# tonyckc/WT-PSE-code

Hardware: AMD Instinct MI355X
Metric: training images/sec (256x256 fundus) — full WT-PSE iteration (higher is better)
Workload: dtype f32 (layers with > 16 output channels and the fused 1x1 heads: x2h (2 fp16 terms per fp32 operand — power-of-two operand scaling —, 3 fp16 MFMA products per multiply, fp32 accumulation); the 16-channel layers the same on 16x16x32, the 1-/3-channel input layers and small 1x1 convs fp32-input MFMA)

## Files before the change

### include/wtpse_hip.h

```cpp
#ifndef WTPSE_HIP_H
#define WTPSE_HIP_H
#ifdef __cplusplus
extern "C" {
#endif


int wtpse_pack_conv_weights(const float* params, const int* desc, int n_desc, float* packed, void* stream);

int wtpse_conv_fwd(const float* in0, int C0, const float* in1, int C1, const float* wpacked, const float* bias,
                   const float* pro0, const float* pro1, int pro_relu, float* out0, float* out1, int Csplit, float* stats,
                   int B, int H, int W, int Cout, int ksize, int relu_out, const float* mask_ref, unsigned* out_amax, void* stream);
int wtpse_conv_stats_blocks(int B, int H, int W);
int wtpse_conv_fwd_gram(const float* in0, int C0, const float* wpacked, const float* bias, const float* pro0, int pro_relu,
                        float* out0, float* gram_partial, int B, int H, int W, int Cout, int relu_out, unsigned* out_amax,
                        void* stream);

int wtpse_conv_x3_stats_blocks(int B, int H, int W, int Cout, int ksize);
int wtpse_x3r_enable(int on);
int wtpse_x3_xcd(int on);
int wtpse_x3_small_wide(int on);
int wtpse_x3_terms(int terms);
int wtpse_amax(const float* x, long long n, unsigned* amax_table, void* stream);
int wtpse_pack_conv_weights_x3(const float* params, const int* desc, int n_desc, unsigned short* packed, void* stream);
int wtpse_conv_fwd_x3(const float* in0, int C0, const float* in1, int C1, const unsigned short* wpacked, const float* bias,
                      const float* pro0, const float* pro1, int pro_relu, float* out0, float* out1, int Csplit, float* stats,
                      int B, int H, int W, int Cout, int ksize, int relu_out, const float* mask_ref, const unsigned* in_amax,
                      const unsigned* in_amax1, unsigned* out_amax, void* stream);

int wtpse_conv16_x3(const float* in0, int C0, const unsigned short* wx16, const float* bias, const float* pro0, int pro_relu,
                    float* out0, float* stats, float* gram_partial, const float* mask_ref, const float* bn_ss,
                    const float* bn_mean, int bn_relu, int B, int H, int W, int Cout, int relu_out, int in_is_grad,
                    const unsigned* in_amax, unsigned* out_amax, void* stream);
int wtpse_pack_conv16_x3(const float* params, const int* desc, int n_desc, unsigned short* packed, void* stream);

int wtpse_dgrad_bnb(const float* dy, int C, const float* wpacked, float* out0, float* out1, int Csplit, const float* bn_y,
                    const float* bn_ss, const float* bn_mean, int bn_relu, int bn_c0, int bn_c1, float* stats, int B, int H, int W,
                    int Cout, int ksize, void* stream);
int wtpse_dgrad_x3_bnb(const float* dy, int C, const unsigned short* wpacked, float* out0, float* out1, int Csplit,
                       const float* bn_y, const float* bn_ss, const float* bn_mean, int bn_relu, int bn_c0, int bn_c1, float* stats,
                       int B, int H, int W, int Cout, int ksize, const unsigned* in_amax, void* stream);

int wtpse_conv_fwd_bnf(const float* in0, int C0, const float* in1, int C1, const void* wpacked, int layout, const float* bias,
                       const float* pro0, const float* pro1, int pro_relu, float* out0, float* stats, const float* gamma,
                       const float* beta, float* running_mean, float* running_var, long long* num_batches, float momentum, float eps,
                       float* scale_shift, float* save_mean, float* save_invstd, double* partial2, unsigned* tickets, int B, int H,
                       int W, int Cout, int ksize, const unsigned* in_amax0, const unsigned* in_amax1, unsigned* act_amax, void* stream);

int wtpse_bnb_tail_partial2(int nblk, int Cout);
int wtpse_bnb_tail_tickets(int nblk, int Cout);
int wtpse_dgrad_bnb_coef(const float* dy, int C, const void* wpacked, int layout, float* out0, float* out1, int Csplit,
                         const float* bn_y, const float* bn_ss, const float* bn_mean, int bn_relu, int bn_c0, int bn_c1,
                         float* stats, const float* gamma, const float* invstd, float* coef, float* dgamma, float* dbeta,
                         int accumulate, double* partial2, unsigned* tickets, int B, int H, int W, int Cout, int ksize,
                         const unsigned* in_amax, void* stream);
int wtpse_dgrad_bnb_coef_frozen(const float* dy, int C, const void* wpacked, int layout, float* out0, float* out1, int Csplit,
                                const float* bn_y, const float* bn_ss, const float* bn_mean, int bn_relu, int bn_c0, int bn_c1,
                                float* stats, const float* gamma, const float* invstd, float* coef, float* dgamma, float* dbeta,
                                float* dbias, int accumulate, double* partial2, unsigned* tickets, int B, int H, int W, int Cout,
                                int ksize, const unsigned* in_amax, void* stream);

int wtpse_conv_wgrad(const float* dy, const float* x0, int C0, const float* x1, int C1, const float* pro0,
                     const float* pro1, int pro_relu, float* slab, float* dbias_slab, int ksplit, float* dw, float* dbias, int accumulate, int B, int H,
                     int W, int Cout, int ksize, void* stream);
int wtpse_wgrad_ksplit(int B, int H, int W, int Cin, int Cout);
int wtpse_wgrad_x3_supported(int Cin, int Cout, int ksize, int C0);
int wtpse_wgrad_x3_ksplit(int B, int H, int W, int Cin, int Cout);
int wtpse_conv_wgrad_x3(const float* dy, const float* x0, int C0, const float* x1, int C1, const float* pro0,
                        const float* pro1, int pro_relu, float* slab, int ksplit, float* dw, int accumulate, int B, int H, int W,
                        int Cout, int ksize, void* stream);

int wtpse_wgrad_r_supported(int Cin, int Cout, int ksize, int C0, int W);
int wtpse_wgrad_r_slabs(int B, int H, int W, int Cin, int Cout);
int wtpse_conv_wgrad_r(const float* dy, const float* x0, int C0, const float* x1, int C1, const float* pro0,
                       const float* pro1, int pro_relu, float* slab, float* dbias_slab, int nslab, float* dw, float* dbias,
                       int accumulate, int B, int H, int W, int Cout, const unsigned* dy_amax, const unsigned* x_amax0,
                       const unsigned* x_amax1, void* stream);

int wtpse_conv_wgrad_r_bn(const float* g, const float* bn_y, const float* bn_coef, const float* x0, int C0, const float* x1,
                          int C1, const float* pro0, const float* pro1, int pro_relu, float* slab, int nslab, float* dw,
                          int accumulate, int B, int H, int W, int Cout, void* stream);

int wtpse_bn_finalize(const float* stats_partial, int nblk, int C, long long count, const float* gamma, const float* beta,
                      float* running_mean, float* running_var, long long* num_batches, float momentum, float eps,
                      float* scale_shift, float* save_mean, float* save_invstd, unsigned* act_amax, void* stream);
int wtpse_bn_finalize_blend(const float* stats_partial, int nblk, int C, long long count, const float* gamma, const float* beta,
                            const float* running_mean, const float* running_var, double w, float eps, double* acc, double acc_count,
                            float* scale_shift, double* moments, double* div, unsigned* act_amax, void* stream);
int wtpse_act_bound(const float* scale_shift, int C, const unsigned* raw_amax, unsigned* act_amax, void* stream);
int wtpse_bn_eval_coeffs(const float* gamma, const float* beta, const float* running_mean, const float* running_var,
                         float eps, int C, float* scale_shift, void* stream);
int wtpse_affine_act(const float* y, const float* scale_shift, int relu, float* z, int B, int C, int HW, void* stream);
int wtpse_bn_bwd(const float* dz, const float* y, const float* scale_shift, int relu, const float* gamma,
                 const float* save_mean, const float* save_invstd, float* partial, float* coef, float* dgamma,
                 float* dbeta, int accumulate, float* dy, int B, int C, int HW, unsigned* amax, void* stream);
int wtpse_bn_bwd_nsplit(int B, int C, int HW);
int wtpse_bn_bwd_reduce(const float* dz, const float* y, const float* scale_shift, int relu, const float* save_mean,
                        const float* save_invstd, float* partial, float* sums_local, int B, int C, int HW, void* stream);
int wtpse_bn_bwd_apply(const float* dz, const float* y, const float* scale_shift, int relu, const float* gamma,
                       const float* save_mean, const float* save_invstd, const float* sums_local, const float* sums_global,
                       long long count_global, float* coef, float* dgamma, float* dbeta, int accumulate, float* dy, int B,
                       int C, int HW, unsigned* amax, void* stream);
int wtpse_bn_bwd_from_stats(const float* g, const float* y, const float* stats_partial, int nblk, const float* gamma,
                            const float* save_mean, const float* save_invstd, float* coef, float* dgamma, float* dbeta,
                            int accumulate, float* dy, int B, int C, int HW, unsigned* amax, void* stream);

int wtpse_bn_bwd_finalize_coef(const float* stats_partial, int nblk, int C, long long count, const float* gamma,
                               const float* save_mean, const float* save_invstd, float* coef, float* dgamma, float* dbeta,
                               int accumulate, void* stream);
int wtpse_bn_bwd_apply_coef(const float* g, const float* y, const float* coef, float* dy, int B, int C, int HW, unsigned* amax, void* stream);

int wtpse_bn_eval_coeffs_stats(const float* gamma, const float* beta, const float* running_mean, const float* running_var,
                               float eps, int C, float* scale_shift, float* save_mean, float* save_invstd, void* stream);
int wtpse_bn_bwd_frozen(const float* dz, const float* y, const float* scale_shift, int relu, const float* gamma,
                        const float* mean, const float* invstd, float* partial, float* coef, float* dgamma, float* dbeta,
                        float* dbias, int accumulate, float* dy, int B, int C, int HW, unsigned* amax, void* stream);
int wtpse_bn_bwd_from_stats_frozen(const float* g, const float* stats_partial, int nblk, const float* gamma, const float* invstd,
                                   float* coef, float* dgamma, float* dbeta, float* dbias, int accumulate, float* dy, int B, int C,
                                   int HW, unsigned* amax, void* stream);
int wtpse_bn_bwd_finalize_coef_frozen(const float* stats_partial, int nblk, int C, const float* gamma, const float* invstd,
                                      float* coef, float* dgamma, float* dbeta, float* dbias, int accumulate, void* stream);
int wtpse_bn_bwd_scale_coef(const float* g, const float* coef, float* dy, int B, int C, int HW, unsigned* amax, void* stream);

int wtpse_wt_loss_fwd(const float* z, int B, int C, int HW, float eps, float margin, int domain_num, int per_domain,
                      float* partial, float* gram, float* v, float* offdiag, float* diag, double* rowval,
                      float* dmmd_dv, float* losses, void* stream);
int wtpse_wt_split(int B, int HW, int* chunk_out);
int wtpse_wt_loss_fwd_partials(const float* partial, int S, int B, int HW, float eps, float margin, int domain_num,
                               int per_domain, float* gram, float* v, float* offdiag, float* diag, double* rowval,
                               float* dmmd_dv, float* losses, void* stream);
// ... 172 lines not shown
```

### wt-pse-code_amd/wtpse_hip/csrc/conv.hip

```cpp
#include "internal.h"

#define WTPSE_P16_KC(KS) ((KS) == 3 ? 4 : 8)

struct ConvArgs {
  const float* in0;
  const float* in1;
  const float* wp;
  const float* bias;
  const float* pro0;
  const float* pro1;
  float* out0;
  float* out1;
  float* stats;
  const float* mask;
  const unsigned* in_amax;
  float in_scale;
  unsigned* out_amax;
  float* gram;
  const float* bn_ss;
  const float* bn_mean;
  int bn_c0, bn_c1, bn_relu;
  BnbTail tail;
  BnfTail ftail;
  int B, H, W;
  int C0, C1, Cin, CinP;
  int Cout, CoutP, Csplit;
  int pro_relu;
  int relu_out;
  int tiles_x, tiles_y;
  int xcd_tiles;
};


template <bool P16> struct AccT { typedef f32x16 type; };
template <> struct AccT<true> { typedef f32x4 type; };
__device__ __forceinline__ f32x4 mfma(float a, float b, f32x4 c) { return mfma16(a, b, c); }
__device__ __forceinline__ f32x16 mfma(float a, float b, f32x16 c) { return mfma32(a, b, c); }

template <int PE>
struct PlaneStride {
  static constexpr int value = ((PE - 16 + 31) / 32) * 32 + 16;
};

template <int KS, int MODE, int TWL, bool DB, int EPI>
__global__ __launch_bounds__(256, 3) void conv_fwd_k(ConvArgs a) {
  constexpr bool MASK = EPI == 1, BNB = EPI == 2;
  constexpr int TAPS = KS * KS, PAD = KS / 2;
  constexpr int TW = 1 << TWL, TH = 256 / TW;
  constexpr int PITCH = TW + 2 * PAD, ROWS = TH + 2 * PAD;
  constexpr int PE = PITCH * ROWS;
  constexpr int NPOS = (PE + 255) / 256;
  constexpr int S = PlaneStride<NPOS * 256>::value;
  constexpr bool XP = (MODE == 3 || MODE == 4);
  constexpr int XT = MODE == 4 ? 2 : 3;
  constexpr bool P16 = (MODE == 0) || XP;
  static_assert(!XP || KS == 3, "MODE 3 / 4 is the 3x3 path");
  constexpr int MT = P16 ? 1 : MODE;
  constexpr int MB = P16 ? 16 : 32;
  constexpr int CB = MB * MT;
  constexpr int NT = P16 ? 4 : 2;
  constexpr int NB = P16 ? 16 : 32;
  constexpr int KC = P16 ? WTPSE_P16_KC(KS) : 8;
  constexpr int KQ = P16 ? 4 : 2;
  constexpr int NACC = P16 ? 4 : 16;
  constexpr int CB4 = CB / 4;
  constexpr int NW = (KC * TAPS * CB4 + 255) / 256;
  constexpr int PEP = (PE + 7) & ~7;
  constexpr int XS_SZ = XP ? 2 * XT * PEP * 4 : KC * S;
  constexpr int WS_SZ = XP ? 0 : NW * 1024;
  constexpr int GRAM_SZ = (P16 && KS == 3) ? 4 * 16 * 65 + 4 * 256 : 0;
  constexpr int RED_SZ = 4 * CB * 2 > GRAM_SZ ? 4 * CB * 2 : GRAM_SZ;
  constexpr int MAIN_SZ = (XS_SZ + WS_SZ) > RED_SZ ? (XS_SZ + WS_SZ) : RED_SZ;
  __shared__ __attribute__((aligned(16))) float smem[MAIN_SZ + CB + (BNB ? 4 * CB : 0)];
  float* bias_s = smem + MAIN_SZ;
  const float* bnp_s = bias_s + CB;
  float* Xs = smem;
  float* Ws = smem + XS_SZ;

  const int tid = threadIdx.x, lane = tid & 63, wave = tid >> 6;
  int tile = (int)blockIdx.x, cblk = (int)blockIdx.y;
  if (a.xcd_tiles > 0) {
    const int L = (int)(blockIdx.y * gridDim.x + blockIdx.x), sl = L >> 3;
    cblk = sl % (int)gridDim.y;
    tile = (L & 7) * a.xcd_tiles + sl / (int)gridDim.y;
  }
  int bx = tile;
  const int tx = bx % a.tiles_x;
  bx /= a.tiles_x;
  const int ty = bx % a.tiles_y;
  const int b = bx / a.tiles_y;
  const int cout0 = cblk * CB;
  const int HW = a.H * a.W;
  if (tid < CB) bias_s[tid] = (a.bias && cout0 + tid < a.Cout) ? a.bias[cout0 + tid] : 0.f;
  if (BNB && tid < CB) bnb_stage<CB>(bias_s + CB + tid, cout0 + tid, a);

  int off[NT];
#pragma unroll
  for (int nt = 0; nt < NT; ++nt) {
    int p = wave * 64 + nt * NB + (lane & (NB - 1));
    off[nt] = (p >> TWL) * PITCH + (p & (TW - 1));
  }

  typename AccT<P16>::type acc[MT][NT];
#pragma unroll
  for (int mt = 0; mt < MT; ++mt)
#pragma unroll
    for (int nt = 0; nt < NT; ++nt)
#pragma unroll
      for (int r = 0; r < NACC; ++r) acc[mt][nt][r] = 0.f;

  if constexpr (XP) {
    u32x4* Xq = reinterpret_cast<u32x4*>(smem);
    const int g4 = lane >> 4;
    constexpr int PB = (PE + 63) / 64, NIT = (2 * PB + 3) / 4;
    const __amdgpu_buffer_rsrc_t rs0 = make_rsrc(a.in0 + (size_t)b * a.C0 * HW, (unsigned)a.C0 * HW * 4u);
    const bool any_pro = MODE == 4 || a.pro0 != nullptr || a.pro_relu != 0;
    const unsigned sx_raw = MODE == 4 ? amax_load(a.in_amax) : 0u;
    __builtin_amdgcn_sched_barrier(0);
    float xv[NIT][8];
    int ipos[NIT], ihalf[NIT];
    bool iin[NIT];
    float psc[2][8], psh[2][8];
#pragma unroll
    for (int hh = 0; hh < 2; ++hh)
#pragma unroll
      for (int j = 0; j < 8; ++j) {
        const int cg = min(hh * 8 + j, a.C0 - 1);
        psc[hh][j] = a.pro0 ? a.pro0[2 * cg] : 1.f;
        psh[hh][j] = a.pro0 ? a.pro0[2 * cg + 1] : 0.f;
      }
#pragma unroll
    for (int i = 0; i < NIT; ++i) {
      const int blk = __builtin_amdgcn_readfirstlane(i * 4 + wave);
      ihalf[i] = blk >= PB ? 1 : 0;
      const int p = (blk - ihalf[i] * PB) * 64 + lane;
      ipos[i] = (blk < 2 * PB && p < PE) ? p : -1;
      const int r = p / PITCH, x = p - r * PITCH;
      const int gy = ty * TH + r - PAD, gx = tx * TW + x - PAD;
      iin[i] = ipos[i] >= 0 && gy >= 0 && gy < a.H && gx >= 0 && gx < a.W;
      const unsigned vo = iin[i] ? (unsigned)(gy * a.W + gx) * 4u : BUF_OOB;
#pragma unroll
      for (int j = 0; j < 8; ++j)
        xv[i][j] = buf_load(rs0, vo, (unsigned)min(ihalf[i] * 8 + j, a.C0) * (unsigned)HW * 4u);
    }
    const u32x4* wq = reinterpret_cast<const u32x4*>(a.wp) + 1 + (MODE == 4 ? 15 * 64 : 0);
    u32x4 afr[5][XT];
#pragma unroll
    for (int s5 = 0; s5 < 5; ++s5)
#pragma unroll
      for (int t = 0; t < XT; ++t) afr[s5][t] = wq[(s5 * XT + t) * 64 + lane];
    const float sx = MODE == 4 ? (a.in_amax ? x3_scale_from_amax(amax_reduce(sx_raw)) : a.in_scale) : 1.f;
    if constexpr (MODE == 4) {
#pragma unroll
      for (int hh = 0; hh < 2; ++hh)
#pragma unroll
        for (int j = 0; j < 8; ++j) {
          psc[hh][j] *= sx;
          psh[hh][j] *= sx;
        }
    }
    if (any_pro) {
      const float lo = (a.pro_relu & 1) ? 0.f : -INFINITY;
#pragma unroll
      for (int i = 0; i < NIT; ++i) {
        const int nc = iin[i] ? a.C0 - ihalf[i] * 8 : 0;
#pragma unroll
        for (int j = 0; j < 8; ++j) {
          const float sc = ihalf[i] ? psc[1][j] : psc[0][j], sh = ihalf[i] ? psh[1][j] : psh[0][j];
          const float v = fmaxf(fmaf(xv[i][j], sc, sh), lo);
          xv[i][j] = j < nc ? v : 0.f;
        }
      }
    }
#pragma unroll
    for (int i = 0; i < NIT; ++i) {
      if (ipos[i] >= 0) {
        u32x4 tt[XT];
#pragma unroll
        for (int j = 0; j < 4; ++j) {
          unsigned q0, q1, q2 = 0u;
          if constexpr (XT == 3) wt_split3_pair(xv[i][2 * j], xv[i][2 * j + 1], q0, q1, q2);
          else split2h_pair(xv[i][2 * j], xv[i][2 * j + 1], q0, q1);
          tt[0][j] = q0; tt[1][j] = q1;
          if constexpr (XT == 3) tt[2][j] = q2;
        }
#pragma unroll
        for (int t = 0; t < XT; ++t) Xq[(t * 2 + ihalf[i]) * PEP + ipos[i]] = tt[t];
      }
    }
    __syncthreads();
    int toff[5];
#pragma unroll
    for (int s5 = 0; s5 < 5; ++s5) {
      const int t = min(2 * s5 + (g4 >> 1), TAPS - 1);
      toff[s5] = (t / KS) * PITCH + (t % KS);
    }
    const int hsel = (g4 & 1) * PEP;
#pragma unroll
    for (int nt = 0; nt < NT; ++nt) {
#pragma unroll
      for (int s5 = 0; s5 < 5; ++s5) {
        u32x4 bfr[XT];
#pragma unroll
        for (int t = 0; t < XT; ++t) bfr[t] = Xq[(t * 2) * PEP + hsel + off[nt] + toff[s5]];
        f32x4 c = acc[0][nt];
        if constexpr (XT == 3) {
          c = wt_mfma16x32(afr[s5][0], bfr[2], c);
          c = wt_mfma16x32(afr[s5][1], bfr[1], c);
          c = wt_mfma16x32(afr[s5][2], bfr[0], c);
          c = wt_mfma16x32(afr[s5][0], bfr[1], c);
          c = wt_mfma16x32(afr[s5][1], bfr[0], c);
          c = wt_mfma16x32(afr[s5][0], bfr[0], c);
        } else {
          c = wt_mfma16x32h(afr[s5][0], bfr[1], c);
          c = wt_mfma16x32h(afr[s5][1], bfr[0], c);
          c = wt_mfma16x32h(afr[s5][0], bfr[0], c);
        }
        acc[0][nt] = c;
      }
    }
    if constexpr (MODE == 4) {
      const float inv = a.wp[0] / sx;
#pragma unroll
      for (int nt = 0; nt < NT; ++nt) acc[0][nt] *= inv;
    }
    __syncthreads();
  } else {
  int gpos[NPOS];
#pragma unroll
  for (int i = 0; i < NPOS; ++i) {
    int p = tid + 256 * i;
    int r = p / PITCH, x = p - r * PITCH;
    int gy = ty * TH + r - PAD, gx = tx * TW + x - PAD;
    gpos[i] = (p < PE && gy >= 0 && gy < a.H && gx >= 0 && gx < a.W) ? gy * a.W + gx : -1;
  }

  const __amdgpu_buffer_rsrc_t rs0 = make_rsrc(a.in0 + (size_t)b * a.C0 * HW, (unsigned)a.C0 * HW * 4u);
  const __amdgpu_buffer_rsrc_t rs1 = a.in1 ? make_rsrc(a.in1 + (size_t)b * a.C1 * HW, (unsigned)a.C1 * HW * 4u) : rs0;
  unsigned voff[NPOS];
#pragma unroll
  for (int i = 0; i < NPOS; ++i) voff[i] = gpos[i] >= 0 ? (unsigned)gpos[i] * 4u : BUF_OOB;
  const __amdgpu_buffer_rsrc_t rsw = make_rsrc(a.wp, (unsigned)a.CinP * TAPS * (unsigned)a.CoutP * 4u);
  unsigned woff[NW];
#pragma unroll
  for (int it = 0; it < NW; ++it) {
    const int e4 = tid + 256 * it;
    const int row = e4 / CB4, j4 = e4 - row * CB4;
    woff[it] = (row < KC * TAPS && cout0 + j4 * 4 < a.CoutP) ? (unsigned)(row * a.CoutP + cout0 + j4 * 4) * 4u : BUF_OOB;
  }
  const bool any_pro = a.pro0 != nullptr || a.pro1 != nullptr || a.pro_relu != 0;
  float xv[KC][NPOS];
  f32x4 wv[NW];
  auto issue_loads = [&](int c0) {
    const bool first = c0 < a.C0;
    const __amdgpu_buffer_rsrc_t rs = first ? rs0 : rs1;
    const int cbase = first ? c0 : c0 - a.C0;
    const int cmax = (first ? a.C0 : a.C1) - 1;
#pragma unroll
    for (int c = 0; c < KC; ++c) {
      const unsigned soff = (unsigned)min(cbase + c, cmax) * (unsigned)HW * 4u;
#pragma unroll
      for (int i = 0; i < NPOS; ++i) xv[c][i] = buf_load(rs, voff[i], soff);
    }
#pragma unroll
    for (int it = 0; it < NW; ++it) wv[it] = buf_load4(rsw, woff[it], (unsigned)(c0 * TAPS) * (unsigned)a.CoutP * 4u);
  };
  auto stash = [&](int c0) {
    const bool first = c0 < a.C0;
    if (any_pro) {
      const bool relu = first ? (a.pro_relu & 1) : (a.pro_relu & 2);
      const float* pro = first ? a.pro0 : a.pro1;
      const int cbase = first ? c0 : c0 - a.C0;
      const int cmax = (first ? a.C0 : a.C1) - 1;
#pragma unroll
      for (int c = 0; c < KC; ++c) {
        const int cg = min(cbase + c, cmax);
        const float sc = pro ? pro[2 * cg] : 1.f, sh = pro ? pro[2 * cg + 1] : 0.f;
#pragma unroll
        for (int i = 0; i < NPOS; ++i) {
          float v = fmaf(xv[c][i], sc, sh);
          if (relu) v = fmaxf(v, 0.f);
          xv[c][i] = gpos[i] >= 0 ? v : 0.f;
        }
      }
    }
#pragma unroll
    for (int c = 0; c < KC; ++c)
#pragma unroll
      for (int i = 0; i < NPOS; ++i) Xs[c * S + tid + 256 * i] = xv[c][i];
#pragma unroll
    for (int it = 0; it < NW; ++it) *reinterpret_cast<f32x4*>(Ws + (tid + 256 * it) * 4) = wv[it];
  };
  if (DB) issue_loads(0);
  for (int c0 = 0; c0 < a.CinP; c0 += KC) {
    const int kc = min(KC, a.CinP - c0);
    __syncthreads();
    if (!DB) issue_loads(c0);
    stash(c0);
    __syncthreads();
    if (DB && c0 + KC < a.CinP) issue_loads(c0 + KC);
    const int nq = kc / KQ;
    for (int q = 0; q < nq; ++q) {
      const int cl = q * KQ + (lane / NB);
      const float* xrow = Xs + cl * S;
      const float* wrow = Ws + cl * TAPS * CB + (lane & (MB - 1));
      float av[TAPS][MT], bv[TAPS][NT];
#pragma unroll
      for (int t = 0; t < TAPS; ++t) {
        const int toff = (t / KS) * PITCH + (t % KS);
#pragma unroll
        for (int mt = 0; mt < MT; ++mt) av[t][mt] = wrow[t * CB + mt * MB];
#pragma unroll
        for (int nt = 0; nt < NT; ++nt) bv[t][nt] = xrow[off[nt] + toff];
      }
#pragma unroll
      for (int t = 0; t < TAPS; ++t)
#pragma unroll
        for (int nt = 0; nt < NT; ++nt)
#pragma unroll
          for (int mt = 0; mt < MT; ++mt) acc[mt][nt] = mfma(av[t][mt], bv[t][nt], acc[mt][nt]);
    }
  }
  }
  if (a.bias) {
    float bz[MT][NACC];
#pragma unroll
    for (int mt = 0; mt < MT; ++mt)
#pragma unroll
      for (int r = 0; r < NACC; ++r)
        bz[mt][r] = bias_s[P16 ? ((lane >> 4) * 4 + r) : (mt * 32 + (r & 3) + 8 * (r >> 2) + 4 * (lane >> 5))];
#pragma unroll
    for (int mt = 0; mt < MT; ++mt)
#pragma unroll
      for (int r = 0; r < NACC; ++r)
#pragma unroll
        for (int nt = 0; nt < NT; ++nt) acc[mt][nt][r] += bz[mt][r];
  }

  const bool want_stats = a.stats != nullptr;
  if (want_stats) __syncthreads();
  float* red = smem;
  const int C1out = a.Cout - a.Csplit;
  int poff[NT];
#pragma unroll
  for (int nt = 0; nt < NT; ++nt) {
    int p = wave * 64 + nt * NB + (lane & (NB - 1));
    int gy = ty * TH + (p >> TWL), gx = tx * TW + (p & (TW - 1));
    poff[nt] = (gy < a.H && gx < a.W) ? gy * a.W + gx : -1;
  }
  const __amdgpu_buffer_rsrc_t rs_o0 = make_rsrc(a.out0 + (size_t)b * a.Csplit * HW, (unsigned)a.Csplit * HW * 4u);
  const __amdgpu_buffer_rsrc_t rs_o1 = a.out1 ? make_rsrc(a.out1 + (size_t)b * C1out * HW, (unsigned)C1out * HW * 4u) : rs_o0;
  const int Cbn = a.bn_c1 - a.bn_c0;
  const __amdgpu_buffer_rsrc_t rs_m = MASK ? make_rsrc(a.mask + (size_t)b * a.Cout * HW, (unsigned)a.Cout * HW * 4u)
                                      : BNB ? make_rsrc(a.mask + (size_t)b * Cbn * HW, (unsigned)Cbn * HW * 4u) : rs_o0;
  const int clane = P16 ? (lane >> 4) * 4 : (lane >> 5) * 4;
  unsigned pvo[NT];
#pragma unroll
  for (int nt = 0; nt < NT; ++nt) pvo[nt] = poff[nt] >= 0 ? (unsigned)(clane * HW + poff[nt]) * 4u : BUF_OOB;
  constexpr int NSV = NACC * 2;
  const bool full = ty * TH + TH <= a.H && tx * TW + TW <= a.W && cout0 + CB <= a.Cout;
  if (!full) {
#pragma unroll
    for (int mt = 0; mt < MT; ++mt)
#pragma unroll
      for (int r = 0; r < NACC; ++r) {
        const bool cvalid = cout0 + (P16 ? r : (mt * 32 + (r & 3) + 8 * (r >> 2))) + clane < a.Cout;
#pragma unroll
        for (int nt = 0; nt < NT; ++nt) acc[mt][nt][r] = (cvalid && poff[nt] >= 0) ? acc[mt][nt][r] : 0.f;
      }
  }
  if (a.relu_out) {
#pragma unroll
    for (int mt = 0; mt < MT; ++mt)
#pragma unroll
      for (int nt = 0; nt < NT; ++nt)
#pragma unroll
        for (int r = 0; r < NACC; ++r) acc[mt][nt][r] = out_clamp<EPI>(acc[mt][nt][r], 0.f);
  }
  if constexpr (P16 && KS == 3) {
    if (a.gram) {
      __syncthreads();
      float* zs = smem + wave * (16 * 65);
#pragma unroll
      for (int nt = 0; nt < NT; ++nt)
#pragma unroll
        for (int r = 0; r < NACC; ++r) zs[((lane >> 4) * 4 + r) * 65 + nt * 16 + (lane & 15)] = acc[0][nt][r];
      __builtin_amdgcn_wave_barrier();
      f32x4 g = {0.f, 0.f, 0.f, 0.f};
#pragma unroll
      for (int st = 0; st < 16; ++st) {
        const float v = zs[(lane & 15) * 65 + 4 * st + (lane >> 4)];
        g = mfma16(v, v, g);
      }
      float* gs = smem + 4 * 16 * 65 + wave * 256;
#pragma unroll
      for (int r = 0; r < 4; ++r) gs[((lane >> 4) * 4 + r) * 16 + (lane & 15)] = g[r];
      __syncthreads();
      const float* g0 = smem + 4 * 16 * 65;
      a.gram[(size_t)tile * 256 + tid] = g0[tid] + g0[256 + tid] + g0[512 + tid] + g0[768 + tid];
      __syncthreads();
    }
  }
  if constexpr (EPI == 0) {
    if (a.out_amax) {
      unsigned am = 0u;
#pragma unroll
      for (int mt = 0; mt < MT; ++mt)
#pragma unroll
        for (int nt = 0; nt < NT; ++nt)
#pragma unroll
          for (int r = 0; r < NACC; ++r) am = max(am, amax_bits(acc[mt][nt][r]));
      amax_publish_wave(a.out_amax, am, (unsigned)tile * 4u + (unsigned)wave);
    }
  }
  const unsigned hw4 = (unsigned)HW * 4u;
  const bool defer = want_stats && (BNB ? a.tail.tickets != nullptr : a.ftail.tickets != nullptr);
#pragma unroll
  for (int mt = 0; mt < MT; ++mt) {
    float mk[NACC][NT];
    if (MASK) {
// ... 51 lines not shown
          if (BNB) {
            const float v = acc[mt][nt][r];
            s1 += v;
            s2 += v * (mk[r][nt] - bmu[r]);
          } else {
            const float v = acc[mt][nt][r];
            s1 += v;
            s2 += v * v;
          }
        }
        sv[r * 2 + 0] = s1;
        sv[r * 2 + 1] = s2;
      }
      constexpr int LB = P16 ? 4 : 5;
      constexpr int HB = P16 ? 3 : 5;
#pragma unroll
      for (int st = 0; st < HB; ++st) {
        const int half = NSV >> (st + 1);
        const bool up = (lane >> st) & 1;
#pragma unroll
        for (int i = 0; i < NSV / 2; ++i) {
          if (i < half) {
            float keep = up ? sv[i + half] : sv[i];
            float send = up ? sv[i] : sv[i + half];
            sv[i] = keep + __shfl_xor(send, 1 << st, 64);
          }
        }
      }
#pragma unroll
      for (int st = HB; st < LB; ++st) sv[0] += __shfl_xor(sv[0], 1 << st, 64);
      int idx = 0;
#pragma unroll
      for (int st = 0; st < HB; ++st) idx += ((lane >> st) & 1) * (NSV >> (st + 1));
      const int k = idx & 1, rr = idx >> 1;
      const int crel = P16 ? ((lane >> 4) * 4 + rr) : (mt * 32 + (rr & 3) + 8 * (rr >> 2) + 4 * (lane >> 5));
      if (((lane & (NB - 1)) >> HB) == 0) red[(wave * CB + crel) * 2 + k] = sv[0];
    }
  }
  if (want_stats) {
    __syncthreads();
    if (tid < CB * 2) {
      int crel = tid >> 1;
      const float s = red[tid] + red[CB * 2 + tid] + red[2 * CB * 2 + tid] + red[3 * CB * 2 + tid];
      if (BNB) {
        const int c = cout0 + crel;
        if (c >= a.bn_c0 && c < a.bn_c1) pub_store(a.stats + ((size_t)tile * Cbn + c - a.bn_c0) * 2 + (tid & 1), s);
      } else if (cout0 + crel < a.Cout) {
        pub_store(a.stats + ((size_t)tile * a.Cout + cout0 + crel) * 2 + (tid & 1), s);
      }
    }
  }
  TailTicket tk;
  tk.old = 0u;
  tk.armed = 0;
  if (defer) {
    if constexpr (BNB) tk = bnb_tail_begin<CB>(a.tail, a.bn_c0, a.bn_c1, cout0, tile, cblk, tid);
    else tk = bnf_tail_begin(a.ftail, tile, cblk, tid);
  }
  if (defer) {
#pragma unroll
    for (int mt = 0; mt < MT; ++mt)
#pragma unroll
      for (int r = 0; r < NACC; ++r) {
        const int cbase = cout0 + (P16 ? r : (mt * 32 + (r & 3) + 8 * (r >> 2)));
        const bool second = a.out1 != nullptr && cbase >= a.Csplit;
        const __amdgpu_buffer_rsrc_t rs_o = second ? rs_o1 : rs_o0;
        const unsigned soff = (unsigned)(second ? min(cbase, a.Cout) - a.Csplit : min(cbase, a.Csplit)) * hw4;
#pragma unroll
        for (int nt = 0; nt < NT; ++nt) buf_store(rs_o, pvo[nt], soff, acc[mt][nt][r]);
      }
    if constexpr (BNB)
      bnb_tail<CB>(tk, a.tail, a.stats, a.bn_mean, a.bn_c0, a.bn_c1, cout0, tile, cblk, tid,
                   reinterpret_cast<double*>(red), reinterpret_cast<int*>(red + 520));
    else
      bnf_tail<CB>(tk, a.ftail, a.stats, a.Cout, cout0, tile, cblk, tid, reinterpret_cast<double*>(red),
                   reinterpret_cast<int*>(red + 520));
  }
}

template <int KS, int MODE, bool DB, int EPI>
static int launch_fwd(const ConvArgs& a, hipStream_t st) {
  constexpr int CB = (MODE == 0 || MODE == 3 || MODE == 4) ? 16 : 32 * MODE;
  ConvArgs args = a;
  const Tiling t = conv_tiling(a.B, a.H, a.W);
  args.tiles_x = t.tiles_x;
  args.tiles_y = t.tiles_y;
  dim3 grid((unsigned)t.tiles, (unsigned)ceil_div(a.CoutP, CB));
  static const bool xcd_on = [] { const char* e = getenv("WTPSE_C16_XCD"); return !(e && e[0] == '0'); }();
  args.xcd_tiles = (xcd_on && grid.x % 8 == 0 && (long long)grid.x * grid.y >= 64) ? (int)(grid.x / 8) : 0;
  const bool in_launch = tail_in_launch((long long)grid.x * grid.y);
  if (!in_launch) args.tail.tickets = args.ftail.tickets = nullptr;
  if (args.tail.tickets) bnb_tail_geometry(args.tail, (int)grid.x, a.Cout, (double)a.B * a.H * a.W);
  if (args.ftail.tickets) bnf_tail_geometry(args.ftail, (int)grid.x, a.Cout, (double)a.B * a.H * a.W);
  if (t.TW == 16)
    hipLaunchKernelGGL((conv_fwd_k<KS, MODE, 4, DB, EPI>), grid, dim3(256), 0, st, args);
  else
    hipLaunchKernelGGL((conv_fwd_k<KS, MODE, 5, DB, EPI>), grid, dim3(256), 0, st, args);
  const int rc = wtpse_status();
  return rc == 0 && !in_launch ? tail_after_launch(a, (int)grid.x, st) : rc;
}

extern "C" int wtpse_conv_stats_blocks(int B, int H, int W) { return conv_tiling(B, H, W).tiles; }

static int conv_check(const ConvCall& c, int layout) {
  const BnbArgs& bn = c.bn;
  const BnbTail& t = c.tail;
  const BnfTail& f = c.ftail;
  const bool bnb = bn.mean != nullptr;
  WTPSE_REQUIRE(layout == CONV_FP32 || layout == CONV_X3 || layout == CONV_C16);
  WTPSE_REQUIRE(c.in0 && c.w && c.out0 && c.B > 0 && c.H > 0 && c.W > 0 && c.C0 > 0 && c.C1 >= 0 && c.Cout > 0);
  WTPSE_REQUIRE(c.ksize == 1 || c.ksize == 3);
  WTPSE_REQUIRE((c.C1 == 0) == (c.in1 == nullptr));
  WTPSE_REQUIRE(c.Csplit > 0 && c.Csplit <= c.Cout && ((c.Csplit == c.Cout) == (c.out1 == nullptr)));
  WTPSE_REQUIRE(c.Csplit == c.Cout || c.Csplit % 16 == 0);
  WTPSE_REQUIRE(!(c.stats && c.relu_out));
  WTPSE_REQUIRE(bnb || !(c.stats && c.mask_ref));
  WTPSE_REQUIRE(bnb || !(c.mask_ref && c.out1));
  WTPSE_REQUIRE(!bnb || (c.mask_ref && c.stats && bn.ss && !c.bias && !c.relu_out && !c.gram && bn.c0 >= 0 && bn.c0 < bn.c1 &&
                         bn.c1 <= c.Cout && bn.c0 % 16 == 0 && (bn.c1 % 16 == 0 || bn.c1 == c.Cout)));
  WTPSE_REQUIRE(c.C1 == 0 || c.C0 % 16 == 0);
  WTPSE_REQUIRE(!(c.out_amax && (c.mask_ref || bnb)));
  WTPSE_REQUIRE(!c.gram || (c.Cout == 16 && !c.relu_out));
  WTPSE_REQUIRE(!t.tickets || (bnb && t.partial2 && t.gamma && t.invstd && t.coef && t.dgamma && t.dbeta));
  WTPSE_REQUIRE(!f.tickets || (!bnb && c.stats && !c.gram && f.partial2 && f.gamma && f.beta && f.scale_shift && f.save_mean &&
                               f.save_invstd && (f.rmean == nullptr) == (f.rvar == nullptr)));
  if (layout == CONV_X3) {
    const X3Tiling g = x3_tiling(c.B, c.H, c.W, c.Cout, c.ksize);
    WTPSE_REQUIRE(!c.gram && !(c.in_amax1 && !c.in1) && ((c.C0 + c.C1 + 15) & ~15) <= (g.mt == 2 && !g.half ? 512 : 256));
  }
  if (layout == CONV_C16)
    WTPSE_REQUIRE(c.ksize == 3 && c.C0 <= 16 && c.Cout <= 16 && (((uintptr_t)c.w) & 15) == 0 && !c.in1 && !c.pro1);
  return 0;
}

static int conv_launch_fwd(const ConvCall& c, bool c16, hipStream_t st) {
  const bool bnb = c.bn.mean != nullptr;
  ConvArgs a;
  a.tail = c.tail;
  a.ftail = c.ftail;
  a.bn_ss = c.bn.ss; a.bn_mean = c.bn.mean; a.bn_relu = c.bn.relu; a.bn_c0 = bnb ? c.bn.c0 : 0; a.bn_c1 = bnb ? c.bn.c1 : 0;
  a.in0 = c.in0; a.in1 = c.in1; a.wp = static_cast<const float*>(c.w); a.bias = c.bias; a.pro0 = c.pro0; a.pro1 = c.pro1;
  a.out0 = c.out0; a.out1 = c.out1; a.stats = c.stats; a.mask = c.mask_ref; a.gram = c.gram;
  a.in_amax = c16 ? c.in_amax0 : nullptr; a.in_scale = c16 ? X3_FWD_SCALE : 1.f; a.out_amax = c.out_amax;
  a.B = c.B; a.H = c.H; a.W = c.W; a.C0 = c.C0; a.C1 = c.C1; a.Cin = c.C0 + c.C1; a.CinP = c16 ? 16 : (a.Cin + 3) & ~3;
  a.Cout = c.Cout; a.CoutP = (c.Cout + 15) & ~15; a.Csplit = c.Csplit; a.pro_relu = c.pro_relu; a.relu_out = c.relu_out;
  a.tiles_x = a.tiles_y = 0;
#define FWD(KS, M, DB) (bnb ? launch_fwd<KS, M, DB, 2>(a, st) : c.mask_ref ? launch_fwd<KS, M, DB, 1>(a, st) : launch_fwd<KS, M, DB, 0>(a, st))
  if (c16) return (g_x3_terms == 2 && (!c.in_is_grad || c.in_amax0)) ? FWD(3, 4, false) : FWD(3, 3, false);
  int mode = c.Cout <= 16 ? 0 : (c.Cout % 64 == 0 ? 2 : 1);
  const int tiles = conv_tiling(c.B, c.H, c.W).tiles;
  if (mode == 2 && tiles * (a.CoutP / 64) < 512) mode = 1;
  if (mode == 1 && tiles * ceil_div(a.CoutP, 32) < 384) mode = 0;
  const int cb = mode == 0 ? 16 : 32 * mode;
  const bool db = tiles * ceil_div(a.CoutP, cb) < 768 && a.CinP > (mode == 0 ? WTPSE_P16_KC(c.ksize) : 8);
#define FWD_DB(KS, M) (db ? FWD(KS, M, true) : FWD(KS, M, false))
  if (c.ksize == 3) return mode == 0 ? FWD_DB(3, 0) : mode == 1 ? FWD_DB(3, 1) : FWD_DB(3, 2);
  return mode == 0 ? FWD_DB(1, 0) : mode == 1 ? FWD_DB(1, 1) : FWD_DB(1, 2);
#undef FWD_DB
#undef FWD
}

int conv_run(const ConvCall& c, int layout, hipStream_t st) {
  if (const int rc = conv_check(c, layout)) return rc;
  return layout == CONV_X3 ? conv_launch_x3(c, st) : conv_launch_fwd(c, layout == CONV_C16, st);
}

extern "C" int wtpse_conv_fwd(const float* in0, int C0, const float* in1, int C1, const float* wpacked,
                              const float* bias, const float* pro0, const float* pro1, int pro_relu, float* out0, float* out1,
                              int Csplit, float* stats, int B, int H, int W, int Cout, int ksize, int relu_out,
                              const float* mask_ref, unsigned* out_amax, void* stream) {
  ConvCall c;
  c.in0 = in0; c.C0 = C0; c.in1 = in1; c.C1 = C1; c.w = wpacked; c.bias = bias; c.pro0 = pro0; c.pro1 = pro1; c.pro_relu = pro_relu;
  c.out0 = out0; c.out1 = out1; c.Csplit = Csplit; c.stats = stats; c.mask_ref = mask_ref; c.out_amax = out_amax;
  c.B = B; c.H = H; c.W = W; c.Cout = Cout; c.ksize = ksize; c.relu_out = relu_out;
  return conv_run(c, CONV_FP32, (hipStream_t)stream);
}

extern "C" int wtpse_dgrad_bnb(const float* dy, int C, const float* wpacked, float* out0, float* out1, int Csplit,
                               const float* bn_y, const float* bn_ss, const float* bn_mean, int bn_relu, int bn_c0, int bn_c1,
                               float* stats, int B, int H, int W, int Cout, int ksize, void* stream) {
  WTPSE_REQUIRE(bn_y && bn_ss && bn_mean && stats);
  ConvCall c;
  c.in0 = dy; c.C0 = C; c.w = wpacked; c.out0 = out0; c.out1 = out1; c.Csplit = Csplit; c.stats = stats; c.mask_ref = bn_y;
  c.bn.ss = bn_ss; c.bn.mean = bn_mean; c.bn.relu = bn_relu; c.bn.c0 = bn_c0; c.bn.c1 = bn_c1;
  c.B = B; c.H = H; c.W = W; c.Cout = Cout; c.ksize = ksize;
  return conv_run(c, CONV_FP32, (hipStream_t)stream);
}

extern "C" int wtpse_conv16_x3(const float* in0, int C0, const unsigned short* wx16, const float* bias, const float* pro0,
                               int pro_relu, float* out0, float* stats, float* gram_partial, const float* mask_ref,
                               const float* bn_ss, const float* bn_mean, int bn_relu, int B, int H, int W, int Cout, int relu_out,
                               int in_is_grad, const unsigned* in_amax, unsigned* out_amax, void* stream) {
  ConvCall c;
  c.in0 = in0; c.C0 = C0; c.w = wx16; c.bias = bias; c.pro0 = pro0; c.pro_relu = pro_relu; c.out0 = out0; c.Csplit = Cout;
  c.stats = stats; c.gram = gram_partial; c.mask_ref = mask_ref; c.in_amax0 = in_amax; c.in_is_grad = in_is_grad; c.out_amax = out_amax;
  c.bn.ss = bn_ss; c.bn.mean = bn_mean; c.bn.relu = bn_relu; c.bn.c1 = Cout;
  c.B = B; c.H = H; c.W = W; c.Cout = Cout; c.ksize = 3; c.relu_out = relu_out;
  return conv_run(c, CONV_C16, (hipStream_t)stream);
}

extern "C" int wtpse_conv_fwd_bnf(const float* in0, int C0, const float* in1, int C1, const void* wpacked, int layout,
                                  const float* bias, const float* pro0, const float* pro1, int pro_relu, float* out0, float* stats,
                                  const float* gamma, const float* beta, float* running_mean, float* running_var,
                                  long long* num_batches, float momentum, float eps, float* scale_shift, float* save_mean,
                                  float* save_invstd, double* partial2, unsigned* tickets, int B, int H, int W, int Cout, int ksize,
                                  const unsigned* in_amax0, const unsigned* in_amax1, unsigned* act_amax, void* stream) {
  WTPSE_REQUIRE(stats && gamma && beta && scale_shift && save_mean && save_invstd && partial2 && tickets);
  ConvCall c;
  c.in0 = in0; c.C0 = C0; c.in1 = in1; c.C1 = C1; c.w = wpacked; c.bias = bias; c.pro0 = pro0; c.pro1 = pro1; c.pro_relu = pro_relu;
  c.out0 = out0; c.Csplit = Cout; c.stats = stats; c.in_amax0 = in_amax0; c.in_amax1 = in_amax1;
  BnfTail& t = c.ftail;
  t.partial2 = partial2; t.tickets = tickets; t.gamma = gamma; t.beta = beta; t.rmean = running_mean; t.rvar = running_var;
  t.nbt = num_batches; t.momentum = momentum; t.eps = eps; t.scale_shift = scale_shift; t.save_mean = save_mean;
  t.save_invstd = save_invstd; t.act_amax = act_amax;
  c.B = B; c.H = H; c.W = W; c.Cout = Cout; c.ksize = ksize;
  return conv_run(c, layout, (hipStream_t)stream);
}

extern "C" int wtpse_bnb_tail_partial2(int nblk, int Cout) { return bnb_tail_groups(nblk) * bnb_tail_ctot(Cout) * 2; }
extern "C" int wtpse_bnb_tail_tickets(int nblk, int Cout) { return bnb_tail_t2off(nblk, Cout) + (Cout + 15) / 16; }

static int dgrad_bnb_coef(ConvCall c, int layout, void* stream) {
  const BnbTail& t = c.tail;
  WTPSE_REQUIRE(c.mask_ref && c.bn.ss && c.bn.mean && c.stats && t.gamma && t.invstd && t.coef && t.dgamma && t.dbeta && t.partial2 &&
                t.tickets);
  c.in_is_grad = 1;
  return conv_run(c, layout, (hipStream_t)stream);
}

extern "C" int wtpse_dgrad_bnb_coef(const float* dy, int C, const void* wpacked, int layout, float* out0, float* out1, int Csplit,
                                    const float* bn_y, const float* bn_ss, const float* bn_mean, int bn_relu, int bn_c0, int bn_c1,
                                    float* stats, const float* gamma, const float* invstd, float* coef, float* dgamma,
                                    float* dbeta, int accumulate, double* partial2, unsigned* tickets, int B, int H, int W,
                                    int Cout, int ksize, const unsigned* in_amax, void* stream) {
  ConvCall c;
  c.in0 = dy; c.C0 = C; c.w = wpacked; c.out0 = out0; c.out1 = out1; c.Csplit = Csplit; c.stats = stats; c.mask_ref = bn_y;
  c.bn.ss = bn_ss; c.bn.mean = bn_mean; c.bn.relu = bn_relu; c.bn.c0 = bn_c0; c.bn.c1 = bn_c1; c.in_amax0 = in_amax;
  BnbTail& t = c.tail;
  t.partial2 = partial2; t.tickets = tickets; t.gamma = gamma; t.invstd = invstd; t.coef = coef; t.dgamma = dgamma; t.dbeta = dbeta;
  t.accumulate = accumulate;
  c.B = B; c.H = H; c.W = W; c.Cout = Cout; c.ksize = ksize;
  return dgrad_bnb_coef(c, layout, stream);
}

extern "C" int wtpse_dgrad_bnb_coef_frozen(const float* dy, int C, const void* wpacked, int layout, float* out0, float* out1,
                                           int Csplit, const float* bn_y, const float* bn_ss, const float* bn_mean, int bn_relu,
                                           int bn_c0, int bn_c1, float* stats, const float* gamma, const float* invstd, float* coef,
                                           float* dgamma, float* dbeta, float* dbias, int accumulate, double* partial2,
                                           unsigned* tickets, int B, int H, int W, int Cout, int ksize, const unsigned* in_amax,
                                           void* stream) {
  WTPSE_REQUIRE(dbias);
  ConvCall c;
  c.in0 = dy; c.C0 = C; c.w = wpacked; c.out0 = out0; c.out1 = out1; c.Csplit = Csplit; c.stats = stats; c.mask_ref = bn_y;
  c.bn.ss = bn_ss; c.bn.mean = bn_mean; c.bn.relu = bn_relu; c.bn.c0 = bn_c0; c.bn.c1 = bn_c1; c.in_amax0 = in_amax;
  BnbTail& t = c.tail;
  t.partial2 = partial2; t.tickets = tickets; t.gamma = gamma; t.invstd = invstd; t.coef = coef; t.dgamma = dgamma; t.dbeta = dbeta;
  t.dbias = dbias; t.accumulate = accumulate;
  c.B = B; c.H = H; c.W = W; c.Cout = Cout; c.ksize = ksize;
  return dgrad_bnb_coef(c, layout, stream);
}

__global__ __launch_bounds__(256) void pack_weights_x3p16_k(const float* __restrict__ params, const int* __restrict__ desc,
                                                            unsigned short* __restrict__ packed) {
  const int* d = desc + blockIdx.y * 8;
  const int w_off = d[0], Co = d[1], Ci = d[2];
  const float* w = params + w_off;
  __shared__ float red[4];
  float m = 0.f;
  for (int e = threadIdx.x; e < Co * Ci * 9; e += 256) m = fmaxf(m, fabsf(w[e]));
  for (int o = 32; o > 0; o >>= 1) m = fmaxf(m, __shfl_xor(m, o, 64));
  if ((threadIdx.x & 63) == 0) red[threadIdx.x >> 6] = m;
  __syncthreads();
  m = fmaxf(fmaxf(red[0], red[1]), fmaxf(red[2], red[3]));
  const float sc = x3_scale_from_amax(__builtin_bit_cast(unsigned, m));
  for (int dir = 0; dir < 2; ++dir) {
    const int base = d[4 + dir];
    if (base < 0) continue;
    const int R = dir == 0 ? Co : Ci, K = dir == 0 ? Ci : Co;
    if (blockIdx.x == 0 && threadIdx.x == 0) {
      float* hdr = reinterpret_cast<float*>(packed + base);
      hdr[0] = 1.f / sc; hdr[1] = sc; hdr[2] = hdr[3] = 0.f;
    }
    for (int e = blockIdx.x * 256 + threadIdx.x; e < 5 * 64 * 8; e += gridDim.x * 256) {
      const int j = e & 7, lane = (e >> 3) & 63, s5 = e >> 9;
      const int row = lane & 15, g = lane >> 4;
      const int tap = 2 * s5 + (g >> 1), k = 8 * (g & 1) + j;
      float v = 0.f;
      if (tap < 9 && row < R && k < K) v = dir == 0 ? w[(row * Ci + k) * 9 + tap] : w[(k * Ci + row) * 9 + (8 - tap)];
      unsigned q0, q1, q2;
      wt_split3_pair(v, 0.f, q0, q1, q2);
      unsigned short* o = packed + base + 8;
      o[((s5 * 3 + 0) * 64 + lane) * 8 + j] = (unsigned short)(q0 & 0xFFFFu);
      o[((s5 * 3 + 1) * 64 + lane) * 8 + j] = (unsigned short)(q1 & 0xFFFFu);
      o[((s5 * 3 + 2) * 64 + lane) * 8 + j] = (unsigned short)(q2 & 0xFFFFu);
      split2h_pair(v * sc, 0.f, q0, q1);
      unsigned short* oh = o + 5 * 3 * 64 * 8;
      oh[((s5 * 2 + 0) * 64 + lane) * 8 + j] = (unsigned short)(q0 & 0xFFFFu);
      oh[((s5 * 2 + 1) * 64 + lane) * 8 + j] = (unsigned short)(q1 & 0xFFFFu);
// ... 423 lines not shown
```

### wt-pse-code_amd/wtpse_hip/csrc/conv_x3.hip

```cpp
#include "conv_x3_kernels.h"

int x3_dispatch_t1(const ConvX3Args& a, const X3Launch& L, hipStream_t st);
int x3_dispatch_t2(const ConvX3Args& a, const X3Launch& L, hipStream_t st);
int x3_dispatch_t3(const ConvX3Args& a, const X3Launch& L, hipStream_t st);

__global__ __launch_bounds__(1024) void pack_scale_x3_k(const float* __restrict__ params, const int* __restrict__ desc,
                                                        unsigned short* __restrict__ packed, int terms) {
  const int* d = desc + blockIdx.y * 8;
  const int n = d[1] * d[2] * d[3];
  const float* w = params + d[0];
  float m = 0.f;
  if (terms == 2)
    for (int e = blockIdx.x * 1024 + threadIdx.x; e < n; e += X3_WSLICES * 1024) m = fmaxf(m, fabsf(w[e]));
  __shared__ float red[16];
  for (int o = 32; o > 0; o >>= 1) m = fmaxf(m, __shfl_xor(m, o, 64));
  if ((threadIdx.x & 63) == 0) red[threadIdx.x >> 6] = m;
  __syncthreads();
  if (threadIdx.x == 0) {
    for (int i = 1; i < 16; ++i) m = fmaxf(m, red[i]);
    reinterpret_cast<float*>(packed + (d[4] >= 0 ? d[4] : d[5]))[4 + blockIdx.x] = m;
  }
}

__global__ __launch_bounds__(256) void pack_weights_x3_k(const float* __restrict__ params, const int* __restrict__ desc,
// ... 44 lines not shown
          split3_pair(v[2 * j], v[2 * j + 1], q0, q1, q2);
        }
        o0[j] = q0; o1[j] = q1; o2[j] = q2;
      }
      const size_t slot = ((((size_t)chunk * (RP / 32) + rb) * T + t) * 6);
      u32x4v* o = reinterpret_cast<u32x4v*>(packed + base + X3_WHDR);
      o[(slot + 0 * 2 + hh) * 32 + row32] = o0;
      o[(slot + 1 * 2 + hh) * 32 + row32] = o1;
      o[(slot + 2 * 2 + hh) * 32 + row32] = o2;
    }
  }
}

int g_x3_terms = [] { const char* e = getenv("WTPSE_X3_TERMS"); return (e && e[0] >= '1' && e[0] <= '3') ? e[0] - '0' : 2; }();
extern "C" int wtpse_x3_terms(int terms) {
  const int was = g_x3_terms;
  if (terms >= 1 && terms <= 3) g_x3_terms = terms;
  return was;
}

extern "C" int wtpse_pack_conv_weights_x3(const float* params, const int* desc, int n_desc, unsigned short* packed, void* stream) {
  WTPSE_REQUIRE(params && desc && packed && n_desc > 0);
  hipLaunchKernelGGL(pack_scale_x3_k, dim3(X3_WSLICES, n_desc), dim3(1024), 0, (hipStream_t)stream, params, desc, packed, g_x3_terms);
  hipLaunchKernelGGL(pack_weights_x3_k, dim3(48, n_desc), dim3(256), 0, (hipStream_t)stream, params, desc, packed, g_x3_terms);
  return wtpse_status();
}

static int g_x3_small_wide = [] { const char* e = getenv("WTPSE_X3_SMALL_WIDE"); return (e && e[0] >= '0' && e[0] <= '1') ? e[0] - '0' : 0; }();
extern "C" int wtpse_x3_small_wide(int on) {
  const int was = g_x3_small_wide;
  if (on >= 0) g_x3_small_wide = on ? 1 : 0;
  return was;
}
static bool x3_small_tiles(int B, int H, int W, int CoutP, bool mt2) {
  if (mt2) return false;
  if (W > 16) return g_x3_small_wide != 0 && W % 32 == 0;
  return conv_tiling(B, H, W).tiles * (CoutP / 32) < 512;
}

static int g_x3r = [] { const char* e = getenv("WTPSE_X3R"); return (e && e[0] >= '0' && e[0] <= '2') ? e[0] - '0' : 1; }();
extern "C" int wtpse_x3r_enable(int on) {
  const int was = g_x3r;
  if (on >= 0) g_x3r = on > 2 ? 2 : on;
  return was;
}

static int g_x3_xcd = [] { const char* e = getenv("WTPSE_X3_XCD"); return (e && e[0] == '0') ? 0 : 1; }();
extern "C" int wtpse_x3_xcd(int on) {
  const int was = g_x3_xcd;
  if (on >= 0) g_x3_xcd = on ? 1 : 0;
  return was;
}

extern "C" int wtpse_tuning_state(void) { return g_x3_terms | (g_x3r << 4) | (g_x3_xcd << 8) | (g_x3_small_wide << 12); }

static bool x3_mt2(int B, int H, int W, int CoutP) {
  const int tiles = conv_tiling(B, H, W).tiles;
  bool mt2 = (CoutP % 64 == 0) && tiles * (CoutP / 64) >= 512;
  static const int mt_override = [] { const char* e = getenv("WTPSE_X3_MT"); return (e && (e[0] == '1' || e[0] == '2')) ? e[0] - '0' : 0; }();
  if (mt_override == 1) mt2 = false;
  if (mt_override == 2 && CoutP % 64 == 0) mt2 = true;
  return mt2;
}

static int g_x3_half_min = [] { const char* e = getenv("WTPSE_X3_HALF"); if (e && e[0] == '0') return 0;
                                const char* m = getenv("WTPSE_X3_HALF_MIN"); const int v = m ? atoi(m) : 256; return v > 0 ? v : 256; }();
static bool x3_half(int B, int H, int W, int CoutP, int ksize, bool mt2) {
  if (ksize != 3 || g_x3_half_min == 0 || g_x3r == 0 || CoutP % 64 != 0 || mt2) return false;
  return conv_tiling(B, H, W, 128).tiles * (CoutP / 64) >= g_x3_half_min;
}

X3Tiling x3_tiling(int B, int H, int W, int Cout, int ksize) {
  const int CoutP = (Cout + 31) & ~31;
  const bool mt2 = x3_mt2(B, H, W, CoutP);
  X3Tiling g;
  g.half = x3_half(B, H, W, CoutP, ksize, mt2) ? 1 : 0;
  g.small = !g.half && x3_small_tiles(B, H, W, CoutP, mt2) ? 1 : 0;
  g.mt = (mt2 || g.half) ? 2 : 1;
  g.px = (g.half || g.small) ? 128 : 256;
  g.t = conv_tiling(B, H, W, g.px);
  return g;
}

extern "C" int wtpse_conv_x3_stats_blocks(int B, int H, int W, int Cout, int ksize) { return x3_tiling(B, H, W, Cout, ksize).t.tiles; }

int conv_launch_x3(const ConvCall& c, hipStream_t st) {
  const bool bnb = c.bn.mean != nullptr;
  ConvX3Args a;
  a.in0 = c.in0; a.in1 = c.in1; a.wx = static_cast<const unsigned short*>(c.w); a.bias = c.bias; a.pro0 = c.pro0; a.pro1 = c.pro1;
  a.out0 = c.out0; a.out1 = c.out1; a.stats = c.stats; a.mask = c.mask_ref;
  a.in_amax = c.in_amax0; a.in_amax1 = c.in_amax1; a.in_scale = X3_FWD_SCALE; a.out_amax = c.out_amax;
  a.bn_ss = c.bn.ss; a.bn_mean = c.bn.mean; a.bn_relu = c.bn.relu; a.bn_c0 = bnb ? c.bn.c0 : 0; a.bn_c1 = bnb ? c.bn.c1 : 0;
  a.tail = c.tail;
  a.ftail = c.ftail;
  a.B = c.B; a.H = c.H; a.W = c.W; a.C0 = c.C0; a.C1 = c.C1; a.Cin = c.C0 + c.C1; a.CinP = (a.Cin + 15) & ~15;
  a.Cout = c.Cout; a.CoutP = (c.Cout + 31) & ~31; a.Csplit = c.Csplit; a.pro_relu = c.pro_relu; a.relu_out = c.relu_out;
  a.tiles_x = a.tiles_y = 0;
  X3Launch L;
  L.g = x3_tiling(c.B, c.H, c.W, c.Cout, c.ksize);
  L.ksize = c.ksize; L.epi = bnb ? 2 : c.mask_ref ? 1 : 0; L.x3r = g_x3r; L.xcd = g_x3_xcd;
  return g_x3_terms == 1 ? x3_dispatch_t1(a, L, st) : g_x3_terms == 2 ? x3_dispatch_t2(a, L, st) : x3_dispatch_t3(a, L, st);
}

extern "C" int wtpse_conv_fwd_x3(const float* in0, int C0, const float* in1, int C1, const unsigned short* wpacked,
                                 const float* bias, const float* pro0, const float* pro1, int pro_relu, float* out0, float* out1,
                                 int Csplit, float* stats, int B, int H, int W, int Cout, int ksize, int relu_out,
                                 const float* mask_ref, const unsigned* in_amax, const unsigned* in_amax1, unsigned* out_amax,
                                 void* stream) {
  ConvCall c;
  c.in0 = in0; c.C0 = C0; c.in1 = in1; c.C1 = C1; c.w = wpacked; c.bias = bias; c.pro0 = pro0; c.pro1 = pro1; c.pro_relu = pro_relu;
  c.out0 = out0; c.out1 = out1; c.Csplit = Csplit; c.stats = stats; c.mask_ref = mask_ref;
  c.in_amax0 = in_amax; c.in_amax1 = in_amax1; c.out_amax = out_amax;
  c.B = B; c.H = H; c.W = W; c.Cout = Cout; c.ksize = ksize; c.relu_out = relu_out;
  return conv_run(c, CONV_X3, (hipStream_t)stream);
}

extern "C" int wtpse_dgrad_x3_bnb(const float* dy, int C, const unsigned short* wpacked, float* out0, float* out1, int Csplit,
                                  const float* bn_y, const float* bn_ss, const float* bn_mean, int bn_relu, int bn_c0, int bn_c1,
                                  float* stats, int B, int H, int W, int Cout, int ksize, const unsigned* in_amax, void* stream) {
  WTPSE_REQUIRE(bn_y && bn_ss && bn_mean && stats);
  ConvCall c;
  c.in0 = dy; c.C0 = C; c.w = wpacked; c.out0 = out0; c.out1 = out1; c.Csplit = Csplit; c.stats = stats; c.mask_ref = bn_y;
  c.bn.ss = bn_ss; c.bn.mean = bn_mean; c.bn.relu = bn_relu; c.bn.c0 = bn_c0; c.bn.c1 = bn_c1; c.in_amax0 = in_amax;
  c.B = B; c.H = H; c.W = W; c.Cout = Cout; c.ksize = ksize;
  return conv_run(c, CONV_X3, (hipStream_t)stream);
}

typedef short s16x4 __attribute__((ext_vector_type(4)));
typedef short s16x8 __attribute__((ext_vector_type(8)));

struct WgradX3Args {
  const float* dy;
  const float* x0;
  const float* x1;
  const float* pro0;
  const float* pro1;
  float* slab;
  int B, H, W, C0, C1, Cin, Cout;
  int pro_relu;
  int tiles_x, tiles_y, ntiles;
  int nci;
};

__device__ __forceinline__ bf16x8 lds_tr8(const u32x4v* base, int byte_off) {
  typedef s16x4 __attribute__((address_space(3))) * lds_p;
  const char __attribute__((address_space(3)))* p =
      (const char __attribute__((address_space(3)))*)base + byte_off;
  const s16x4 lo = __builtin_amdgcn_ds_read_tr16_b64_v4i16((lds_p)p);
  const s16x4 hi = __builtin_amdgcn_ds_read_tr16_b64_v4i16((lds_p)(p + 64));
  const s16x8 v = __builtin_shufflevector(lo, hi, 0, 1, 2, 3, 4, 5, 6, 7);
  return __builtin_bit_cast(bf16x8, v);
}

constexpr int pad_plane(int n) {
  for (int m = n;; ++m)
    if (m % 16 == 4 || m % 16 == 12) return m;
}

#define WSPLIT(a, b, q0, q1, q2) split3_pair(a, b, q0, q1, q2)
#define WSTORE(dst, v) dst = v
template <int KS, int TWL, bool Q>
__global__ __launch_bounds__(256, 2) void conv_wgrad_x3_k(WgradX3Args a) {
  constexpr int TAPS = KS * KS, PAD = KS / 2;
  constexpr int NPX = Q ? 64 : 128;
  constexpr int TW = 1 << TWL, TH = NPX >> TWL;
  constexpr int PITCH = TW + 2 * PAD, ROWS = TH + 2 * PAD;
  constexpr int PE = PITCH * ROWS;
  constexpr int NCG = Q ? 8 : 4;
  constexpr int BLK = NCG * 8;
  constexpr int XP = pad_plane(PE), YP = pad_plane(NPX);
  constexpr int XS_U4 = 3 * NCG * XP, YS_U4 = 3 * NCG * YP;
  constexpr int RED_U4 = Q ? 0 : 4 * 1024 / 4;
  constexpr int SM_U4 = (XS_U4 + YS_U4) > RED_U4 ? (XS_U4 + YS_U4) : RED_U4;
  __shared__ u32x4v smem[SM_U4];
  u32x4v* Xs = smem;
  u32x4v* Ys = smem + XS_U4;

  const int tid = threadIdx.x, lane = tid & 63, wave = tid >> 6;
  int bx = blockIdx.x, ky = blockIdx.y;
  if ((gridDim.y & 7) == 0) {
    const int lin = blockIdx.y * gridDim.x + blockIdx.x;
    const int k = lin >> 3;
    ky = (lin & 7) + 8 * (k / (int)gridDim.x);
// ... 236 lines not shown
```

### wt-pse-code_amd/wtpse_hip/csrc/conv_x3_kernels.h

```cpp
#pragma once

#include <stdlib.h>
#include "internal.h"
#include <utility>

typedef __bf16 bf16x8 __attribute__((ext_vector_type(8)));
typedef __bf16 bf16x2 __attribute__((ext_vector_type(2)));
typedef unsigned int u32x4v __attribute__((ext_vector_type(4)));

struct ConvX3Args {
  const float* in0;
  const float* in1;
  const unsigned short* wx;
  const float* bias;
  const float* pro0;
  const float* pro1;
  float* out0;
  float* out1;
  float* stats;
  const float* mask;
  const unsigned* in_amax;
  const unsigned* in_amax1;
  float in_scale;
  unsigned* out_amax;
  const float* bn_ss;
  const float* bn_mean;
  int bn_c0, bn_c1, bn_relu;
  BnbTail tail;
  BnfTail ftail;
  int B, H, W;
  int C0, C1, Cin, CinP;
  int Cout, CoutP, Csplit;
  int pro_relu, relu_out;
  int tiles_x, tiles_y;
  int xcd_tiles;
};

__device__ __forceinline__ void x3_block_ids(const ConvX3Args& a, int& tile, int& cblk) {
  tile = blockIdx.x;
  cblk = blockIdx.y;
  if (a.xcd_tiles > 0) {
    const int L = blockIdx.y * gridDim.x + blockIdx.x, s = L >> 3;
    cblk = s % (int)gridDim.y;
    tile = (L & 7) * a.xcd_tiles + s / (int)gridDim.y;
  }
}

template <class F, int... I>
__device__ __forceinline__ void x3_static_for_impl(F&& f, std::integer_sequence<int, I...>) {
  (f(std::integral_constant<int, I>{}), ...);
}
template <int N, class F>
__device__ __forceinline__ void x3_static_for(F&& f) {
  x3_static_for_impl(f, std::make_integer_sequence<int, N>{});
}

__device__ __forceinline__ f32x16 mfma_bf16(bf16x8 a, bf16x8 b, f32x16 c) {
  return __builtin_amdgcn_mfma_f32_32x32x16_bf16(a, b, c, 0, 0, 0);
}

template <int TERMS>
__device__ __forceinline__ unsigned x3_in_scale_issue(const ConvX3Args& a) {
  if constexpr (TERMS != 2) return 0u;
  else return max(amax_load(a.in_amax), amax_load(a.in_amax1));
}
template <int TERMS>
__device__ __forceinline__ float x3_in_scale(const ConvX3Args& a, unsigned issued) {
  if constexpr (TERMS != 2) return 1.f;
  else {
    if (!a.in_amax && !a.in_amax1) return a.in_scale;
    return x3_scale_from_amax(amax_reduce(issued));
  }
}

__device__ __forceinline__ unsigned pack_rne(float a, float b) {
  bf16x2 v = {(__bf16)a, (__bf16)b};
  return __builtin_bit_cast(unsigned, v);
}
__device__ __forceinline__ void split3_pair(float a, float b, unsigned& p0, unsigned& p1, unsigned& p2) {
  p0 = pack_rne(a, b);
  const float ra = a - __builtin_bit_cast(float, p0 << 16);
  const float rb = b - __builtin_bit_cast(float, p0 & 0xFFFF0000u);
  p1 = pack_rne(ra, rb);
  const float sa = ra - __builtin_bit_cast(float, p1 << 16);
  const float sb = rb - __builtin_bit_cast(float, p1 & 0xFFFF0000u);
  p2 = pack_rne(sa, sb);
// ... 150 lines not shown
        float s1 = 0.f, s2 = 0.f;
#pragma unroll
        for (int nt = 0; nt < NT; ++nt) {
#pragma clang fp contract(off)
          if (BNB) {
            const float v = acc[mt][nt][r];
            s1 += v;
            s2 += v * (mk[r][nt] - bmu[r]);
          } else {
            const float v = acc[mt][nt][r];
            s1 += v;
            s2 += v * v;
          }
        }
        sv[r * 2 + 0] = s1;
        sv[r * 2 + 1] = s2;
      }
#pragma unroll
      for (int st = 0; st < 5; ++st) {
        const int half = NSV >> (st + 1);
        const bool up = (lane >> st) & 1;
#pragma unroll
        for (int i = 0; i < NSV / 2; ++i) {
          if (i < half) {
            float lo = sv[i], hi = sv[i + half];
            asm volatile("" : "+v"(lo), "+v"(hi));
            const float keep = up ? hi : lo;
            const float send = up ? lo : hi;
            sv[i] = keep + __shfl_xor(send, 1 << st, 64);
          }
        }
      }
      int idx = 0;
#pragma unroll
      for (int st = 0; st < 5; ++st) idx += ((lane >> st) & 1) * (NSV >> (st + 1));
      const int k = idx & 1, rr = idx >> 1;
      const int crel = cw0 + mt * 32 + (rr & 3) + 8 * (rr >> 2) + 4 * h;
      red[(wave * CB + crel) * 2 + k] = sv[0];
    }
  }
  if (want_stats) {
    __syncthreads();
    if (tid < CB * 2) {
      const int crel = tid >> 1;
      float s = red[tid];
#pragma unroll
      for (int q = 1; q < PW; ++q) s += red[q * CB * 2 + tid];
      if (BNB) {
        const int c = cout0 + crel;
        if (live && c >= a.bn_c0 && c < a.bn_c1) pub_store(a.stats + ((size_t)stats_row * Cbn + c - a.bn_c0) * 2 + (tid & 1), s);
      } else if (live && cout0 + crel < a.Cout) {
        pub_store(a.stats + ((size_t)stats_row * a.Cout + cout0 + crel) * 2 + (tid & 1), s);
      }
    }
  }
  TailTicket tk;
  tk.old = 0u;
  tk.armed = 0;
  if (defer) {
    if constexpr (BNB) tk = bnb_tail_begin<CB>(a.tail, a.bn_c0, a.bn_c1, cout0, stats_row, cblk, tid);
    else tk = bnf_tail_begin(a.ftail, stats_row, cblk, tid);
  }
  if (defer) {
#pragma unroll
    for (int mt = 0; mt < MT; ++mt)
#pragma unroll
      for (int r = 0; r < NACC; ++r) {
        const int cbase = cout0 + cw0 + mt * 32 + (r & 3) + 8 * (r >> 2);
        const bool second = a.out1 != nullptr && cbase >= a.Csplit;
        const __amdgpu_buffer_rsrc_t rs_o = second ? rs_o1 : rs_o0;
        const unsigned soff = (unsigned)(second ? min(cbase, a.Cout) - a.Csplit : min(cbase, a.Csplit)) * hw4;
#pragma unroll
        for (int nt = 0; nt < NT; ++nt) buf_store(rs_o, pvo[nt], soff, acc[mt][nt][r]);
      }
    if constexpr (BNB)
      bnb_tail<CB>(tk, a.tail, a.stats, a.bn_mean, a.bn_c0, a.bn_c1, cout0, stats_row, cblk, tid,
                   reinterpret_cast<double*>(red), reinterpret_cast<int*>(red + 520));
    else
      bnf_tail<CB>(tk, a.ftail, a.stats, a.Cout, cout0, stats_row, cblk, tid, reinterpret_cast<double*>(red),
                   reinterpret_cast<int*>(red + 520));
  }
}

template <int KS, int MT, int TWL, int EPI, int NT = 2, int TERMS = 3>
__global__ __launch_bounds__(256, 2) void conv_x3_k(ConvX3Args a) {
  static_assert(TERMS >= 1 && TERMS <= 3, "three bf16 terms (x3), two fp16 terms (x2h) or one bf16 term (bf16 mode)");
  constexpr int TAPS = KS * KS, PAD = KS / 2;
  constexpr int TW = 1 << TWL, TH = (128 * NT) / TW;
  constexpr int PITCH = TW + 2 * PAD, ROWS = TH + 2 * PAD;
  constexpr int PE = PITCH * ROWS;
  constexpr int PEP = (PE + 7) & ~7;
  constexpr int CB = 32 * MT;
  constexpr int NACC = 16;
  constexpr int KC = 16;
  constexpr int XS_U4 = 2 * TERMS * PEP;
  constexpr int WS_U4 = KS * 2 * TERMS * CB;
  constexpr int NW = (WS_U4 + 255) / 256;
  constexpr int RED_F = 4 * CB * 2;
  constexpr int MAIN_U4 = (XS_U4 + 2 * WS_U4) > (RED_F + 3) / 4 ? (XS_U4 + 2 * WS_U4) : (RED_F + 3) / 4;
  constexpr int PRO_MAX = MT == 1 ? 256 : 512;
  __shared__ u32x4v smem[MAIN_U4 + CB / 4 + (EPI == 2 ? CB : 0)];
  __shared__ float2 pro_s[PRO_MAX];
  u32x4v* Xs = smem;
  u32x4v* Ws = smem + XS_U4;
  float* bias_s = reinterpret_cast<float*>(smem + MAIN_U4);

  const int tid = threadIdx.x, lane = tid & 63, wave = tid >> 6;
  const int r32 = lane & 31, h = lane >> 5;
  int tile, cblk;
  x3_block_ids(a, tile, cblk);
  int bx = tile;
  const int tx = bx % a.tiles_x;
  bx /= a.tiles_x;
  const int ty = bx % a.tiles_y;
  const int b = bx / a.tiles_y;
  const int cout0 = cblk * CB;
  const int HW = a.H * a.W;
  if (tid < CB) bias_s[tid] = (a.bias && cout0 + tid < a.Cout) ? a.bias[cout0 + tid] : 0.f;
  if (EPI == 2 && tid < CB) bnb_stage<CB>(bias_s + CB + tid, cout0 + tid, a);

  float sx = 1.f;

  int off[NT];
#pragma unroll
  for (int nt = 0; nt < NT; ++nt) {
    const int p = wave * (32 * NT) + nt * 32 + r32;
    off[nt] = (p >> TWL) * PITCH + (p & (TW - 1));
  }
  constexpr int PB = (PE + 63) / 64;
  constexpr int NIT = (2 * PB + 3) / 4;
  int ipos[NIT], ihalf[NIT];
  unsigned voff[NIT];
  bool iin[NIT];
#pragma unroll
  for (int i = 0; i < NIT; ++i) {
    const int blk = __builtin_amdgcn_readfirstlane(i * 4 + wave);
    ihalf[i] = blk >= PB ? 1 : 0;
    const int p = (blk - ihalf[i] * PB) * 64 + lane;
    ipos[i] = (blk < 2 * PB && p < PE) ? p : -1;
    const int r = p / PITCH, x = p - r * PITCH;
    const int gy = ty * TH + r - PAD, gx = tx * TW + x - PAD;
    iin[i] = ipos[i] >= 0 && gy >= 0 && gy < a.H && gx >= 0 && gx < a.W;
    voff[i] = iin[i] ? (unsigned)(gy * a.W + gx) * 4u + (unsigned)ihalf[i] * 8u * (unsigned)HW * 4u : BUF_OOB;
  }

  f32x16 acc[MT][NT];
#pragma unroll
  for (int mt = 0; mt < MT; ++mt)
#pragma unroll
    for (int nt = 0; nt < NT; ++nt)
#pragma unroll
      for (int r = 0; r < NACC; ++r) acc[mt][nt][r] = 0.f;

  const __amdgpu_buffer_rsrc_t rs0 = make_rsrc(a.in0 + (size_t)b * a.C0 * HW, (unsigned)a.C0 * HW * 4u);
  const __amdgpu_buffer_rsrc_t rs1 = a.in1 ? make_rsrc(a.in1 + (size_t)b * a.C1 * HW, (unsigned)a.C1 * HW * 4u) : rs0;
  const int ncb32 = a.CoutP / 32;
  const __amdgpu_buffer_rsrc_t rsw = make_rsrc(a.wx + X3_WHDR, (unsigned)(a.CinP / 16) * ncb32 * TAPS * 6u * 32u * 16u);

  float xv[NIT][8];
  u32x4v wv[NW];
  auto issue_x = [&](int c0) {
    const bool first = c0 < a.C0;
    const __amdgpu_buffer_rsrc_t rs = first ? rs0 : rs1;
    const int cbase = first ? c0 : c0 - a.C0;
    const int cn = first ? a.C0 : a.C1;
#pragma unroll
    for (int j = 0; j < 8; ++j) {
      const unsigned soff = (unsigned)min(cbase + j, cn) * (unsigned)HW * 4u;
#pragma unroll
      for (int i = 0; i < NIT; ++i) xv[i][j] = buf_load(rs, voff[i], soff);
    }
  };
  u32x4v tq[NIT][TERMS];
  const bool any_pro = a.pro0 != nullptr || a.pro1 != nullptr || a.pro_relu != 0;
  auto convert_pair = [&](int c0, int i, int j, bool pro) __attribute__((always_inline)) {
    float v0 = xv[i][2 * j], v1 = xv[i][2 * j + 1];
    if (pro) {
      const float lo = ((c0 < a.C0) ? (a.pro_relu & 1) : (a.pro_relu & 2)) ? 0.f : -INFINITY;
      const int cg = min(c0 + ihalf[i] * 8 + 2 * j, PRO_MAX - 2);
      const float2 p0 = pro_s[cg], p1 = pro_s[cg + 1];
      v0 = fmaxf(fmaf(v0, p0.x, p0.y), lo);
      v1 = fmaxf(fmaf(v1, p1.x, p1.y), lo);
      v0 = iin[i] ? v0 : 0.f;
      v1 = iin[i] ? v1 : 0.f;
    } else if (TERMS == 2) {
      v0 *= sx;
      v1 *= sx;
    }
    unsigned q[TERMS];
    x3_split_pair<TERMS>(v0, v1, q);
#pragma unroll
    for (int t = 0; t < TERMS; ++t) tq[i][t][j] = q[t];
  };
  auto store_x = [&]() __attribute__((always_inline)) {
#pragma unroll
    for (int i = 0; i < NIT; ++i) {
      if (ipos[i] >= 0) {
#pragma unroll
        for (int t = 0; t < TERMS; ++t) Xs[(t * 2 + ihalf[i]) * PEP + ipos[i]] = tq[i][t];
      }
    }
  };
  auto stash_x = [&](int c0) __attribute__((always_inline)) {
    if (any_pro) x3_static_for<NIT * 4>([&](auto pc) __attribute__((always_inline)) { convert_pair(c0, decltype(pc)::value >> 2, decltype(pc)::value & 3, true); });
    else x3_static_for<NIT * 4>([&](auto pc) __attribute__((always_inline)) { convert_pair(c0, decltype(pc)::value >> 2, decltype(pc)::value & 3, false); });
    store_x();
  };
  unsigned wslot[NW];
#pragma unroll
  for (int it = 0; it < NW; ++it) {
    const int s = tid + 256 * it;
    const int co = s % CB, q6 = (s / CB) % (2 * TERMS), tl = s / (CB * 2 * TERMS);
    const bool ok = s < WS_U4 && cout0 + co < a.CoutP;
    wslot[it] = ok ? (unsigned)(((co >> 5) * (TAPS * 6 * 32) + (tl * 6 + q6) * 32 + (co & 31)) * 16) : BUF_OOB;
  }
  auto issue_w = [&](int chunk, int ky) {
    const unsigned base = ((unsigned)(chunk * ncb32 + cout0 / 32) * (unsigned)(TAPS * 6 * 32) + (unsigned)(ky * KS * 6 * 32)) * 16u;
#pragma unroll
    for (int it = 0; it < NW; ++it) wv[it] = __builtin_bit_cast(u32x4v, buf_load4(rsw, wslot[it], base));
  };
  auto stash_w = [&](int buf) {
#pragma unroll
    for (int it = 0; it < NW; ++it)
      if (NW * 256 == WS_U4 || tid + 256 * it < WS_U4) Ws[buf * WS_U4 + tid + 256 * it] = wv[it];
// ... 50 lines not shown
      {
        u32x4v a01[2][MT][2], a2[MT], bfr[NT][3];
        auto rd_a = [&](int tl, int t) {
#pragma unroll
          for (int mt = 0; mt < MT; ++mt) {
            const u32x4v v = Wb[((tl * 2 * TERMS) + t * 2 + h) * CB + mt * 32 + r32];
            if (t == 2) a2[mt] = v; else a01[tl & 1][mt][t] = v;
          }
        };
        auto rd_b = [&](int tl, int t) {
#pragma unroll
          for (int nt = 0; nt < NT; ++nt) bfr[nt][t] = Xs[(t * 2 + h) * PEP + off[nt] + ky * PITCH + tl];
        };
        auto mm = [&](int tl, int ta, int tb) {
#pragma unroll
          for (int mt = 0; mt < MT; ++mt)
#pragma unroll
            for (int nt = 0; nt < NT; ++nt) acc[mt][nt] = x3_mfma<TERMS>(ta == 2 ? a2[mt] : a01[tl & 1][mt][ta], bfr[nt][tb], acc[mt][nt]);
        };
        if constexpr (TERMS == 1) {
          rd_a(0, 0); rd_b(0, 0);
#pragma unroll
          for (int tl = 0; tl < KS; ++tl) {
            mm(tl, 0, 0);
            if (tl + 1 < KS) { rd_a(tl + 1, 0); rd_b(tl + 1, 0); }
          }
        } else if constexpr (TERMS == 2) {
          rd_a(0, 0); rd_b(0, 1); rd_a(0, 1); rd_b(0, 0);
#pragma unroll
          for (int tl = 0; tl < KS; ++tl) {
            const bool nx = tl + 1 < KS;
            __builtin_amdgcn_sched_barrier(0);
            mm(tl, 0, 1);
            if (nx) { rd_b(tl + 1, 1); rd_a(tl + 1, 0); }
            __builtin_amdgcn_sched_barrier(0);
            mm(tl, 1, 0);
            if (nx) rd_a(tl + 1, 1);
            __builtin_amdgcn_sched_barrier(0);
            mm(tl, 0, 0);
            if (nx) rd_b(tl + 1, 0);
          }
        } else {
        rd_a(0, 0); rd_b(0, 2); rd_a(0, 1); rd_b(0, 1); rd_a(0, 2); rd_b(0, 0);
#pragma unroll
        for (int tl = 0; tl < KS; ++tl) {
          const bool nx = tl + 1 < KS;
          __builtin_amdgcn_sched_barrier(0);
          mm(tl, 0, 2);
          if (nx) { rd_b(tl + 1, 2); rd_a(tl + 1, 0); }
          convert_piece();
          __builtin_amdgcn_sched_barrier(0);
          mm(tl, 1, 1);
          if (nx) rd_a(tl + 1, 1);
          convert_piece();
          __builtin_amdgcn_sched_barrier(0);
          mm(tl, 2, 0);
          if (nx) rd_a(tl + 1, 2);
          convert_piece();
          __builtin_amdgcn_sched_barrier(0);
          mm(tl, 0, 1);
          if (nx) rd_b(tl + 1, 1);
          convert_piece();
          __builtin_amdgcn_sched_barrier(0);
          mm(tl, 1, 0);
          convert_piece();
          __builtin_amdgcn_sched_barrier(0);
          mm(tl, 0, 0);
          if (nx) rd_b(tl + 1, 0);
          convert_piece();
        }
        }
      }
      __builtin_amdgcn_sched_barrier(0);
      if (more) stash_w(buf ^ 1);
      if (last_row && more) {
        __syncthreads();
        if (PIPE) store_x(); else stash_x((chunk + 1) * KC);
      }
      __syncthreads();
      buf ^= 1;
    }
  }
  x3_unscale<TERMS, MT, NT>(a, acc, sx);
  x3_epilogue<MT, NT, TWL, EPI, true>(a, acc, b, ty, tx, cout0, tid, reinterpret_cast<float*>(smem), bias_s, tile, cblk, true);
}


template <int WM, int MT, int NT, int TWL, int EPI, int TERMS = 3, bool PLAIN = false>
__global__ __launch_bounds__(256, 2) void conv_x3r_k(ConvX3Args a) {
  static_assert(TERMS >= 1 && TERMS <= 3, "three bf16 terms (x3), two fp16 terms (x2h) or one bf16 term (bf16 mode)");
  constexpr int KS = 3, TAPS = 9, PAD = 1;
  constexpr int PW = 4 / WM;
  constexpr int TW = 1 << TWL, TH = (PW * 32 * NT) / TW;
  constexpr int PITCH = TW + 2 * PAD, ROWS = TH + 2 * PAD;
  constexpr int PE = PITCH * ROWS;
  constexpr int PEP = (PE + 7) & ~7;
  constexpr int CBW = 32 * MT, CB = CBW * WM;
  constexpr int NACC = 16;
  constexpr int KC = 16;
  constexpr int XS_U4 = 2 * TERMS * PEP;
  constexpr int MAIN_U4 = 2 * XS_U4;
  constexpr int PRO_MAX = 512;
  static_assert(MAIN_U4 * 4 >= PW * CB * 2 + 4 * CB + 4 && MAIN_U4 * 4 >= 524, "epilogue scratch (statistics, the tails' 256 doubles + flag) aliases the operand images");
  constexpr int DUMP_U4 = MAIN_U4 + CB / 4 + (EPI == 2 ? CB : 0);
  __shared__ u32x4v smem[DUMP_U4 + 64];
  __shared__ float2 pro_s[PRO_MAX];
  u32x4v* Xs = smem;
  float* bias_s = reinterpret_cast<float*>(smem + MAIN_U4);

  const int tid = threadIdx.x, lane = tid & 63, wave = tid >> 6;
  const int cw = __builtin_amdgcn_readfirstlane(wave % WM), pw = __builtin_amdgcn_readfirstlane(wave / WM);
  const int r32 = lane & 31, h = lane >> 5;
  int tile, cblk;
  x3_block_ids(a, tile, cblk);
  int bx = tile;
  const int tx = bx % a.tiles_x;
  bx /= a.tiles_x;
  const int ty = bx % a.tiles_y;
  const int b = bx / a.tiles_y;
  const int cout0 = cblk * CB;
  const int HW = a.H * a.W;
  float sx = 1.f;
  if (tid < CB) bias_s[tid] = (a.bias && cout0 + tid < a.Cout) ? a.bias[cout0 + tid] : 0.f;
  if (EPI == 2 && tid < CB) bnb_stage<CB>(bias_s + CB + tid, cout0 + tid, a);

  int off[NT];
#pragma unroll
  for (int nt = 0; nt < NT; ++nt) {
    const int p = pw * (32 * NT) + nt * 32 + r32;
    off[nt] = (p >> TWL) * PITCH + (p & (TW - 1));
  }
  constexpr int PB = (PE + 63) / 64;
  constexpr int NIT = (2 * PB + 3) / 4;
  int ipos[NIT], ihalf[NIT];
  unsigned voff[NIT];
  bool iin[NIT];
#pragma unroll
  for (int i = 0; i < NIT; ++i) {
    const int blk = __builtin_amdgcn_readfirstlane(i * 4 + wave);
    ihalf[i] = blk >= PB ? 1 : 0;
    const int p = (blk - ihalf[i] * PB) * 64 + lane;
    ipos[i] = (blk < 2 * PB && p < PE) ? p : -1;
    const int r = p / PITCH, x = p - r * PITCH;
    const int gy = ty * TH + r - PAD, gx = tx * TW + x - PAD;
    iin[i] = ipos[i] >= 0 && gy >= 0 && gy < a.H && gx >= 0 && gx < a.W;
    voff[i] = iin[i] ? (unsigned)(gy * a.W + gx) * 4u + (unsigned)ihalf[i] * 8u * (unsigned)HW * 4u : BUF_OOB;
  }

  f32x16 acc[MT][NT];
#pragma unroll
  for (int mt = 0; mt < MT; ++mt)
#pragma unroll
    for (int nt = 0; nt < NT; ++nt)
#pragma unroll
      for (int r = 0; r < NACC; ++r) acc[mt][nt][r] = 0.f;

  const int ncb32 = a.CoutP / 32;
  const int nchunks = a.CinP / KC;
  constexpr unsigned TAP_B = 6u * 32u * 16u;
  const __amdgpu_buffer_rsrc_t rsw = make_rsrc(a.wx + X3_WHDR, (unsigned)nchunks * ncb32 * TAPS * TAP_B);
  const unsigned wlane = (unsigned)lane * 16u;
  const int cb32 = cout0 / 32 + cw * MT;

  float xv[NIT][8];
  const float* const xb0 = a.in0 + (size_t)b * a.C0 * HW;
  const float* const xb1 = a.in1 ? a.in1 + (size_t)b * a.C1 * HW : xb0;
  auto issue_x = [&](int c0) __attribute__((always_inline)) {
// ... 74 lines not shown

  constexpr int NPIECE = NIT * 4;
  constexpr int NGRP = TAPS * NT;
  static_assert(NPIECE <= NGRP, "one conversion piece per MFMA group");
  constexpr int G0 = NGRP - NPIECE;

  if constexpr (PLAIN) {
    sx = x3_in_scale<TERMS>(a, x3_in_scale_issue<TERMS>(a));
    issue_x(0);
    issue_a(0, 0, 0);
    issue_a(0, 1, 1);
  } else {
    float2 praw[PRO_MAX / 256];
#pragma unroll
    for (int q = 0; q < PRO_MAX / 256; ++q) {
      const int c = tid + 256 * q;
      const bool first = c < a.C0;
      const float* pro = first ? a.pro0 : a.pro1;
      const int cl = first ? c : c - a.C0;
      const bool live = c < a.C0 + a.C1;
      praw[q] = !live ? make_float2(0.f, 0.f) : (pro ? make_float2(pro[2 * cl], pro[2 * cl + 1]) : make_float2(1.f, 0.f));
    }
    const unsigned sx_raw = x3_in_scale_issue<TERMS>(a);
    __builtin_amdgcn_sched_barrier(0);
    issue_x(0);
    issue_a(0, 0, 0);
    issue_a(0, 1, 1);
    sx = x3_in_scale<TERMS>(a, sx_raw);
#pragma unroll
    for (int q = 0; q < PRO_MAX / 256; ++q)
      if (tid + 256 * q < a.CinP) pro_s[tid + 256 * q] = make_float2(praw[q].x * sx, praw[q].y * sx);
  }
  __syncthreads();
  x3_static_for<NPIECE>([&](auto pc) __attribute__((always_inline)) { convert_piece(0, decltype(pc)::value, 0); });
  issue_x(KC);
  __syncthreads();
  for (int chunk = 0; chunk < nchunks; ++chunk) {
    const int xb = chunk & 1;
    const int chn = min(chunk + 1, nchunks - 1);
    const int c0n = (chunk + 1) * KC;
    __builtin_amdgcn_sched_barrier(0);
    rd_b(xb, 0, 0, 0);
    x3_static_for<NGRP>([&](auto gc) __attribute__((always_inline)) {
      constexpr int g = decltype(gc)::value;
      constexpr int tap = g / NT, nt = g % NT;
      __builtin_amdgcn_sched_barrier(0);
      if constexpr (nt == 0) {
        if constexpr (tap + 2 < TAPS) issue_a(chunk, tap + 2, (tap + 2) % 3);
        else issue_a(chn, tap + 2 - TAPS, (tap + 2) % 3);
      }
      if constexpr (g + 1 < NGRP) rd_b(xb, (g + 1) / NT, (g + 1) % NT, (g + 1) & 1);
      __builtin_amdgcn_sched_barrier(0);
      mm(tap % RING, nt, g & 1);
      if constexpr (g >= G0) convert_piece(c0n, g - G0, xb ^ 1);
    });
    __builtin_amdgcn_sched_barrier(0);
    issue_x((chunk + 2) * KC);
    __syncthreads();
  }
  x3_unscale<TERMS, MT, NT>(a, acc, sx);
  x3_epilogue<MT, NT, TWL, EPI, true, WM>(a, acc, b, ty, tx, cout0, tid, reinterpret_cast<float*>(smem), bias_s, tile, cblk, true);
}


struct X3Launch {
  X3Tiling g;
  int ksize;
  int epi;
  int x3r;
  int xcd;
};

template <int KS, int MT, int EPI, int TERMS>
static int launch_x3(const ConvX3Args& a, const X3Launch& L, hipStream_t st) {
  ConvX3Args args = a;
  const bool narrow = L.g.t.TW == 16, half = L.g.half != 0, small = L.g.small != 0;
  args.tiles_x = L.g.t.tiles_x;
  args.tiles_y = L.g.t.tiles_y;
  dim3 grid((unsigned)L.g.t.tiles, (unsigned)ceil_div(a.CoutP, 32 * MT));
  args.xcd_tiles = (L.xcd && grid.x % 8 == 0 && (long long)grid.x * grid.y >= 64) ? (int)grid.x / 8 : 0;
  const bool in_launch = tail_in_launch((long long)grid.x * grid.y);
  if (!in_launch) args.tail.tickets = args.ftail.tickets = nullptr;
  if (args.tail.tickets) bnb_tail_geometry(args.tail, (int)grid.x, a.Cout, (double)a.B * a.H * a.W);
  if (args.ftail.tickets) bnf_tail_geometry(args.ftail, (int)grid.x, a.Cout, (double)a.B * a.H * a.W);
  if (KS == 3 && (L.x3r == 2 || (L.x3r == 1 && MT == 2))) {
    if constexpr (KS == 3) {
      const bool plain = !a.pro0 && !a.pro1 && !a.pro_relu;
#define X3R_GO(WM_, NT_, TWL_)                                                                                          \
  do {                                                                                                                  \
    if (plain) hipLaunchKernelGGL((conv_x3r_k<WM_, 1, NT_, TWL_, EPI, TERMS, true>), grid, dim3(256), 0, st, args);     \
    else hipLaunchKernelGGL((conv_x3r_k<WM_, 1, NT_, TWL_, EPI, TERMS, false>), grid, dim3(256), 0, st, args);          \
  } while (0)
      if (half) {
        if constexpr (MT == 2) {
          if (narrow) X3R_GO(2, 2, 4);
          else X3R_GO(2, 2, 5);
        }
      } else if (small) {
        if constexpr (MT == 1) {
          if (narrow) X3R_GO(1, 1, 4);
          else X3R_GO(1, 1, 5);
        }
      } else if (MT == 2) {
        if (narrow) X3R_GO(2, 4, 4);
        else X3R_GO(2, 4, 5);
      } else {
        if (narrow) X3R_GO(1, 2, 4);
        else X3R_GO(1, 2, 5);
      }
#undef X3R_GO
    }
  } else if (small) {
    if constexpr (MT == 1) {
      if (narrow) hipLaunchKernelGGL((conv_x3_k<KS, 1, 4, EPI, 1, TERMS>), grid, dim3(256), 0, st, args);
      else hipLaunchKernelGGL((conv_x3_k<KS, 1, 5, EPI, 1, TERMS>), grid, dim3(256), 0, st, args);
    }
  } else if (narrow)
    hipLaunchKernelGGL((conv_x3_k<KS, MT, 4, EPI, 2, TERMS>), grid, dim3(256), 0, st, args);
  else
    hipLaunchKernelGGL((conv_x3_k<KS, MT, 5, EPI, 2, TERMS>), grid, dim3(256), 0, st, args);
  const int rc = wtpse_status();
  return rc == 0 && !in_launch ? tail_after_launch(a, (int)grid.x, st) : rc;
}

template <int TERMS>
static int x3_dispatch(const ConvX3Args& a, const X3Launch& L, hipStream_t st) {
#define X3E(KS, M) (L.epi == 2 ? launch_x3<KS, M, 2, TERMS>(a, L, st) : L.epi == 1 ? launch_x3<KS, M, 1, TERMS>(a, L, st) : launch_x3<KS, M, 0, TERMS>(a, L, st))
  if (L.ksize == 3) return L.g.mt == 2 ? X3E(3, 2) : X3E(3, 1);
  return L.g.mt == 2 ? X3E(1, 2) : X3E(1, 1);
#undef X3E
}
```

### wt-pse-code_amd/wtpse_hip/csrc/internal.h

```cpp
#pragma once
#include <cstdlib>
#include "common.h"

#define WTPSE_INTERNAL __attribute__((visibility("hidden")))

WTPSE_INTERNAL extern int g_x3_terms;

struct BnbArgs {
  const float* ss = nullptr;
  const float* mean = nullptr;
  int relu = 0, c0 = 0, c1 = 0;
};
struct ConvCall {
  const float* in0 = nullptr; int C0 = 0;
  const float* in1 = nullptr; int C1 = 0;
  const void* w = nullptr;
  const float* bias = nullptr;
  const float* pro0 = nullptr; const float* pro1 = nullptr; int pro_relu = 0;
  float* out0 = nullptr; float* out1 = nullptr; int Csplit = 0;
  float* stats = nullptr;
  const float* mask_ref = nullptr;
  float* gram = nullptr;
  const unsigned* in_amax0 = nullptr; const unsigned* in_amax1 = nullptr;
  int in_is_grad = 0;
  unsigned* out_amax = nullptr;
  BnbArgs bn;
  BnbTail tail = bnb_tail_none();
  BnfTail ftail = bnf_tail_none();
  int B = 0, H = 0, W = 0, Cout = 0, ksize = 0, relu_out = 0;
};
enum { CONV_FP32 = 0, CONV_X3 = 1, CONV_C16 = 2 };
WTPSE_INTERNAL int conv_run(const ConvCall& c, int layout, hipStream_t st);
WTPSE_INTERNAL int conv_launch_x3(const ConvCall& c, hipStream_t st);

struct Tiling {
  int TW, TH, tiles_x, tiles_y, tiles;
};
static inline Tiling make_tiling(int B, int H, int W, bool narrow, int pixels) {
  Tiling t;
  t.TW = narrow ? 16 : 32; t.TH = pixels / t.TW;
  t.tiles_x = ceil_div(W, t.TW); t.tiles_y = ceil_div(H, t.TH); t.tiles = B * t.tiles_x * t.tiles_y;
  return t;
}
static inline Tiling conv_tiling(int B, int H, int W, int pixels = 256) { return make_tiling(B, H, W, W <= 16, pixels); }
struct X3Tiling {
  int mt;
  int px;
  int half;
  int small;
  Tiling t;
};
WTPSE_INTERNAL X3Tiling x3_tiling(int B, int H, int W, int Cout, int ksize);

struct WgradCall {
  const float* dy = nullptr;
  const float* x0 = nullptr; int C0 = 0;
  const float* x1 = nullptr; int C1 = 0;
  const float* pro0 = nullptr; const float* pro1 = nullptr; int pro_relu = 0;
  float* slab = nullptr; float* dbias_slab = nullptr; int nslab = 0;
  float* dw = nullptr; float* dbias = nullptr; int accumulate = 0;
  const float* bn_y = nullptr; const float* bn_coef = nullptr; const unsigned* dy_amax = nullptr;
  const unsigned* x_amax0 = nullptr; const unsigned* x_amax1 = nullptr;
  int B = 0, H = 0, W = 0, Cout = 0, ksize = 0;
};
enum { WGRAD_FP32 = 0, WGRAD_X3 = 1, WGRAD_R = 2 };
WTPSE_INTERNAL int wgrad_run(const WgradCall& c, int family, hipStream_t st);
WTPSE_INTERNAL int wgrad_launch_x3(const WgradCall& c, hipStream_t st);
WTPSE_INTERNAL int wgrad_launch_r(const WgradCall& c, hipStream_t st);

struct WgradX3Geometry {
  Tiling t;
  int q, blk, nci, nx, ksplit;
};
WTPSE_INTERNAL WgradX3Geometry wgrad_x3_geometry(int B, int H, int W, int Cin, int Cout);
struct WgradRPlan {
  int mf, nf, nw, pairs, nci, wpp, nseg, rseg, units, strips, nslab;
};
WTPSE_INTERNAL bool wgrad_r_plan(int B, int H, int W, int Cin, int Cout, WgradRPlan& p);

static inline bool tail_in_launch(long long workgroups) {
  static const long long max_wgs = [] { const char* e = getenv("WTPSE_TAIL_MAX_WGS"); return e ? atoll(e) : 8192ll; }();
  return workgroups <= max_wgs;
}
template <class Args>
static inline int tail_after_launch(const Args& a, int nblk, hipStream_t stream) {
  const BnbTail& tl = a.tail;
  const BnfTail& fl = a.ftail;
  const long long count = (long long)a.B * a.H * a.W;
  if (tl.tickets && tl.dbias)
    return wtpse_bn_bwd_finalize_coef_frozen(a.stats, nblk, a.bn_c1 - a.bn_c0, tl.gamma, tl.invstd, tl.coef, tl.dgamma, tl.dbeta,
                                             tl.dbias, tl.accumulate, stream);
  if (tl.tickets)
    return wtpse_bn_bwd_finalize_coef(a.stats, nblk, a.bn_c1 - a.bn_c0, count, tl.gamma, a.bn_mean, tl.invstd, tl.coef, tl.dgamma,
                                      tl.dbeta, tl.accumulate, stream);
  if (fl.tickets)
    return wtpse_bn_finalize(a.stats, nblk, a.Cout, count, fl.gamma, fl.beta, fl.rmean, fl.rvar, fl.nbt, fl.momentum, fl.eps,
                             fl.scale_shift, fl.save_mean, fl.save_invstd, fl.act_amax, stream);
  return 0;
}
```

### wt-pse-code_amd/wtpse_hip/csrc/pointwise.hip

```cpp
#include "common.h"

__device__ __forceinline__ float act_in(float v, const float* pro, int c, int relu) {
  if (pro) v = fmaf(v, pro[2 * c], pro[2 * c + 1]);
  return relu ? fmaxf(v, 0.f) : v;
}

__device__ __forceinline__ float block_sum(float v, float* sh4) {
  v = wave_xor_sum(v, 32);
  __syncthreads();
  if ((threadIdx.x & 63) == 0) sh4[threadIdx.x >> 6] = v;
  __syncthreads();
  return sh4[0] + sh4[1] + sh4[2] + sh4[3];
}

__global__ __launch_bounds__(256) void maxpool2_fwd_k(const float* __restrict__ x, const float* __restrict__ pro, int relu,
                                                      float* __restrict__ out, int C, int H, int W, long long total) {
  const int Ho = H / 2, Wo = W / 2;
  long long i = (long long)blockIdx.x * 256 + threadIdx.x;
  if (i >= total) return;
  int xo = (int)(i % Wo);
  long long r = i / Wo;
  int yo = (int)(r % Ho);
  long long bc = r / Ho;
  int c = (int)(bc % C);
  const float* src = x + (size_t)bc * H * W + (size_t)(2 * yo) * W + 2 * xo;
  float a = act_in(src[0], pro, c, relu), b = act_in(src[1], pro, c, relu);
  float d = act_in(src[W], pro, c, relu), e = act_in(src[W + 1], pro, c, relu);
  out[i] = fmaxf(fmaxf(a, b), fmaxf(d, e));
}

__global__ __launch_bounds__(256) void maxpool2_fwd_v_k(const float* __restrict__ x, const float* __restrict__ pro, int relu,
                                                        float* __restrict__ out, int BC, int C, int H, int W) {
  const int Ho = H / 2, Wo = W / 2, W4 = W / 4;
  const int j = blockIdx.x * 256 + threadIdx.x;
  if (j >= Ho * W4) return;
  const int k = j % W4, yo = j / W4;
  for (int bc = blockIdx.y; bc < BC; bc += gridDim.y) {
    const int c = bc % C;
    const float* src = x + (size_t)bc * H * W + (size_t)(2 * yo) * W + 4 * k;
    const float4 r0 = *reinterpret_cast<const float4*>(src), r1 = *reinterpret_cast<const float4*>(src + W);
    float2 o;
    o.x = fmaxf(fmaxf(act_in(r0.x, pro, c, relu), act_in(r0.y, pro, c, relu)), fmaxf(act_in(r1.x, pro, c, relu), act_in(r1.y, pro, c, relu)));
    o.y = fmaxf(fmaxf(act_in(r0.z, pro, c, relu), act_in(r0.w, pro, c, relu)), fmaxf(act_in(r1.z, pro, c, relu), act_in(r1.w, pro, c, relu)));
    *reinterpret_cast<float2*>(out + (size_t)bc * Ho * Wo + (size_t)yo * Wo + 2 * k) = o;
  }
}

__device__ __forceinline__ int pool_argmax(float v0, float v1, float v2, float v3) {
  int am = 0;
  float m = v0;
  if (v1 > m || isnan(v1)) { m = v1; am = 1; }
  if (v2 > m || isnan(v2)) { m = v2; am = 2; }
  if (v3 > m || isnan(v3)) { m = v3; am = 3; }
  return am;
}

__global__ __launch_bounds__(256) void maxpool2_bwd_v_k(const float* __restrict__ x, const float* __restrict__ pro, int relu,
                                                        const float* __restrict__ dout, float* __restrict__ dx, int accumulate,
                                                        int BC, int C, int H, int W, const float* __restrict__ mean,
                                                        float* __restrict__ stats) {
  __shared__ float sh4[4];
  const int Ho = H / 2, Wo = W / 2, W4 = W / 4;
  const int jj = blockIdx.x * 256 + threadIdx.x;
  const bool valid = jj < Ho * W4;
  if (!valid && !stats) return;
  const int j = valid ? jj : 0;
  const int k = j % W4, yo = j / W4;
  for (int bc = blockIdx.y; bc < BC; bc += gridDim.y) {
    const int c = bc % C;
    const size_t off = (size_t)bc * H * W + (size_t)(2 * yo) * W + 4 * k;
    const float4 r0 = *reinterpret_cast<const float4*>(x + off), r1 = *reinterpret_cast<const float4*>(x + off + W);
    const float2 g = *reinterpret_cast<const float2*>(dout + (size_t)bc * Ho * Wo + (size_t)yo * Wo + 2 * k);
    const int a0 = pool_argmax(act_in(r0.x, pro, c, relu), act_in(r0.y, pro, c, relu), act_in(r1.x, pro, c, relu), act_in(r1.y, pro, c, relu));
    const int a1 = pool_argmax(act_in(r0.z, pro, c, relu), act_in(r0.w, pro, c, relu), act_in(r1.z, pro, c, relu), act_in(r1.w, pro, c, relu));
    float4 d0 = make_float4(a0 == 0 ? g.x : 0.f, a0 == 1 ? g.x : 0.f, a1 == 0 ? g.y : 0.f, a1 == 1 ? g.y : 0.f);
    float4 d1 = make_float4(a0 == 2 ? g.x : 0.f, a0 == 3 ? g.x : 0.f, a1 == 2 ? g.y : 0.f, a1 == 3 ? g.y : 0.f);
    if (accumulate & 1) {
      const float4 p0 = *reinterpret_cast<const float4*>(dx + off), p1 = *reinterpret_cast<const float4*>(dx + off + W);
      d0 = make_float4(p0.x + d0.x, p0.y + d0.y, p0.z + d0.z, p0.w + d0.w);
      d1 = make_float4(p1.x + d1.x, p1.y + d1.y, p1.z + d1.z, p1.w + d1.w);
    }
    if (accumulate & 2) {
      d0.x = act_in(r0.x, pro, c, relu) > 0.f ? d0.x : 0.f; d0.y = act_in(r0.y, pro, c, relu) > 0.f ? d0.y : 0.f;
      d0.z = act_in(r0.z, pro, c, relu) > 0.f ? d0.z : 0.f; d0.w = act_in(r0.w, pro, c, relu) > 0.f ? d0.w : 0.f;
      d1.x = act_in(r1.x, pro, c, relu) > 0.f ? d1.x : 0.f; d1.y = act_in(r1.y, pro, c, relu) > 0.f ? d1.y : 0.f;
      d1.z = act_in(r1.z, pro, c, relu) > 0.f ? d1.z : 0.f; d1.w = act_in(r1.w, pro, c, relu) > 0.f ? d1.w : 0.f;
    }
    if (valid) {
      *reinterpret_cast<float4*>(dx + off) = d0;
      *reinterpret_cast<float4*>(dx + off + W) = d1;
    }
    if (stats) {
      const float mu = mean[c];
      float s1 = 0.f, s2 = 0.f;
      if (valid) {
#pragma clang fp contract(off)
        s1 = ((d0.x + d0.y) + (d0.z + d0.w)) + ((d1.x + d1.y) + (d1.z + d1.w));
        s2 = ((d0.x * (r0.x - mu) + d0.y * (r0.y - mu)) + (d0.z * (r0.z - mu) + d0.w * (r0.w - mu))) +
             ((d1.x * (r1.x - mu) + d1.y * (r1.y - mu)) + (d1.z * (r1.z - mu) + d1.w * (r1.w - mu)));
      }
      s1 = block_sum(s1, sh4);
      s2 = block_sum(s2, sh4);
      if (threadIdx.x == 0) {
        float* dst = stats + (((size_t)(bc / C) * gridDim.x + blockIdx.x) * C + c) * 2;
        dst[0] = s1;
        dst[1] = s2;
      }
    }
  }
}

__global__ __launch_bounds__(256) void maxpool2_bwd_k(const float* __restrict__ x, const float* __restrict__ pro, int relu,
                                                      const float* __restrict__ dout, float* __restrict__ dx,
                                                      int accumulate, int C, int H, int W, long long total) {
  const int Ho = H / 2, Wo = W / 2;
  long long i = (long long)blockIdx.x * 256 + threadIdx.x;
  if (i >= total) return;
  int xx = (int)(i % W);
  long long r = i / W;
  int yy = (int)(r % H);
  long long bc = r / H;
  int c = (int)(bc % C);
  float g = 0.f;
  int yo = yy >> 1, xo = xx >> 1;
  if (yo < Ho && xo < Wo) {
    const float* src = x + (size_t)bc * H * W + (size_t)(2 * yo) * W + 2 * xo;
    float v[4] = {act_in(src[0], pro, c, relu), act_in(src[1], pro, c, relu), act_in(src[W], pro, c, relu),
                  act_in(src[W + 1], pro, c, relu)};
    int am = 0;
    float m = v[0];
#pragma unroll
    for (int k = 1; k < 4; ++k)
      if (v[k] > m || isnan(v[k])) { m = v[k]; am = k; }
    if (am == (yy & 1) * 2 + (xx & 1)) g = dout[(size_t)bc * Ho * Wo + (size_t)yo * Wo + xo];
  }
  g = (accumulate & 1) ? dx[i] + g : g;
  if ((accumulate & 2) && !(act_in(x[i], pro, c, relu) > 0.f)) g = 0.f;
  dx[i] = g;
}

__device__ __forceinline__ void up_src(int d, int n, int& i0, int& i1, float& l1) {
  float s = 0.5f * (d + 0.5f) - 0.5f;
  if (s < 0.f) s = 0.f;
  i0 = (int)s;
  i1 = i0 + (i0 < n - 1 ? 1 : 0);
  l1 = s - (float)i0;
}

__global__ __launch_bounds__(256) void upsample2x_fwd_k(const float* __restrict__ x, const float* __restrict__ pro, int relu,
                                                        float* __restrict__ out, int C, int H, int W, long long total) {
  const int Ho = 2 * H, Wo = 2 * W;
  long long i = (long long)blockIdx.x * 256 + threadIdx.x;
  if (i >= total) return;
  int xo = (int)(i % Wo);
  long long r = i / Wo;
  int yo = (int)(r % Ho);
  long long bc = r / Ho;
  int c = (int)(bc % C);
  int y0, y1, x0, x1;
  float ly, lx;
  up_src(yo, H, y0, y1, ly);
  up_src(xo, W, x0, x1, lx);
  const float* src = x + (size_t)bc * H * W;
  float v00 = act_in(src[y0 * W + x0], pro, c, relu), v01 = act_in(src[y0 * W + x1], pro, c, relu);
  float v10 = act_in(src[y1 * W + x0], pro, c, relu), v11 = act_in(src[y1 * W + x1], pro, c, relu);
  const float h0 = lx < 0.5f ? fmaf(lx, v01, (1.f - lx) * v00) : fmaf(1.f - lx, v00, lx * v01);
  const float h1 = lx < 0.5f ? fmaf(lx, v11, (1.f - lx) * v10) : fmaf(1.f - lx, v10, lx * v11);
  out[i] = fmaf(1.f - ly, h0, ly * h1);
}

__device__ __forceinline__ float up_w(int d, int n, int k) {
  int i0, i1;
  float l1;
  up_src(d, n, i0, i1, l1);
  return (i0 == k ? 1.f - l1 : 0.f) + (i1 == k ? l1 : 0.f);
}

__global__ __launch_bounds__(256) void upsample2x_fwd4_v_k(const float* __restrict__ x, const float* __restrict__ pro, int relu,
                                                           float* __restrict__ out, float* __restrict__ stats, int BC, int C,
                                                           int H, int W) {
  __shared__ float sh4[4];
  const int Ho = 2 * H, Wo = 2 * W, W2 = W / 2;
  const int jj = blockIdx.x * 256 + threadIdx.x;
  const bool valid = jj < (H + 1) * W2;
  if (!valid && !stats) return;
  const int j = valid ? jj : 0;
  const int k = j % W2, p = j / W2 - 1;
  const int ya = 2 * p + 1, yb = 2 * p + 2;
  const bool va = valid && ya >= 0, vb = valid && yb < Ho;
  int t0, t1;
  float la = 0.f, lb = 0.f;
  if (ya >= 0) up_src(ya, H, t0, t1, la);
  if (yb < Ho) up_src(yb, H, t0, t1, lb);
  const int y0 = max(p, 0), y1 = p < 0 ? min(1, H - 1) : min(p + 1, H - 1);
  const int m = 2 * k;
  const int xm1 = max(m - 1, 0), x1 = min(m + 1, W - 1), x2 = min(m + 2, W - 1);
  for (int bc = blockIdx.y; bc < BC; bc += gridDim.y) {
    const int c = bc % C;
    const float* r0 = x + (size_t)bc * H * W + (size_t)y0 * W;
    const float* r1 = x + (size_t)bc * H * W + (size_t)y1 * W;
    float a[4] = {act_in(r0[xm1], pro, c, relu), act_in(r0[m], pro, c, relu), act_in(r0[x1], pro, c, relu), act_in(r0[x2], pro, c, relu)};
    float b[4] = {act_in(r1[xm1], pro, c, relu), act_in(r1[m], pro, c, relu), act_in(r1[x1], pro, c, relu), act_in(r1[x2], pro, c, relu)};
    float ha[4], hb[4];
    if (m == 0) { ha[0] = fmaf(0.f, a[2], a[1]); hb[0] = fmaf(0.f, b[2], b[1]); }
    else        { ha[0] = fmaf(0.25f, a[0], 0.75f * a[1]); hb[0] = fmaf(0.25f, b[0], 0.75f * b[1]); }
    ha[1] = fmaf(0.25f, a[2], 0.75f * a[1]); hb[1] = fmaf(0.25f, b[2], 0.75f * b[1]);
    ha[2] = fmaf(0.25f, a[1], 0.75f * a[2]); hb[2] = fmaf(0.25f, b[1], 0.75f * b[2]);
    ha[3] = fmaf(0.25f, a[3], 0.75f * a[2]); hb[3] = fmaf(0.25f, b[3], 0.75f * b[2]);
    float4 oa, ob;
    oa.x = fmaf(1.f - la, ha[0], la * hb[0]);
    oa.y = fmaf(1.f - la, ha[1], la * hb[1]);
    oa.z = fmaf(1.f - la, ha[2], la * hb[2]);
    oa.w = fmaf(1.f - la, ha[3], la * hb[3]);
    ob.x = fmaf(1.f - lb, ha[0], lb * hb[0]);
    ob.y = fmaf(1.f - lb, ha[1], lb * hb[1]);
    ob.z = fmaf(1.f - lb, ha[2], lb * hb[2]);
    ob.w = fmaf(1.f - lb, ha[3], lb * hb[3]);
    float* ob0 = out + (size_t)bc * Ho * Wo + 4 * k;
    if (va) *reinterpret_cast<float4*>(ob0 + (size_t)ya * Wo) = oa;
    if (vb) *reinterpret_cast<float4*>(ob0 + (size_t)yb * Wo) = ob;
    if (stats) {
      float s1 = (va ? (oa.x + oa.y) + (oa.z + oa.w) : 0.f) + (vb ? (ob.x + ob.y) + (ob.z + ob.w) : 0.f);
      float s2 = (va ? (oa.x * oa.x + oa.y * oa.y) + (oa.z * oa.z + oa.w * oa.w) : 0.f) +
                 (vb ? (ob.x * ob.x + ob.y * ob.y) + (ob.z * ob.z + ob.w * ob.w) : 0.f);
      s1 = block_sum(s1, sh4);
      s2 = block_sum(s2, sh4);
      if (threadIdx.x == 0) {
        float* dst = stats + (((size_t)(bc / C) * gridDim.x + blockIdx.x) * C + c) * 2;
        dst[0] = s1;
        dst[1] = s2;
      }
    }
  }
}

__global__ __launch_bounds__(256) void upsample2x_bwd_k(const float* __restrict__ dout, float* __restrict__ dx,
                                                        int accumulate, int H, int W, long long total) {
  const int Ho = 2 * H, Wo = 2 * W;
  long long i = (long long)blockIdx.x * 256 + threadIdx.x;
  if (i >= total) return;
  int xx = (int)(i % W);
  long long r = i / W;
  int yy = (int)(r % H);
  long long bc = r / H;
  const float* src = dout + (size_t)bc * Ho * Wo;
  float g = 0.f;
#pragma unroll
  for (int dy = -1; dy <= 2; ++dy) {
    int yo = 2 * yy + dy;
    if (yo < 0 || yo >= Ho) continue;
    float wy = up_w(yo, H, yy);
    if (wy == 0.f) continue;
    float rowsum = 0.f;
#pragma unroll
    for (int dxo = -1; dxo <= 2; ++dxo) {
      int xo = 2 * xx + dxo;
      if (xo < 0 || xo >= Wo) continue;
      float wx = up_w(xo, W, xx);
      rowsum += wx * src[(size_t)yo * Wo + xo];
    }
    g += wy * rowsum;
  }
  dx[i] = accumulate ? dx[i] + g : g;
}

template <bool BN>
__global__ __launch_bounds__(256) void upsample2x_bwd_v_k(const float* __restrict__ dout, float* __restrict__ dx, int accumulate,
                                                          int BC, int H, int W, const float* __restrict__ bn_y,
                                                          const float* __restrict__ bn_coef, int C, unsigned* __restrict__ amax) {
  const int Ho = 2 * H, Wo = 2 * W, W4 = W / 4;
  const int j = blockIdx.x * 256 + threadIdx.x;
  const bool live = j < H * W4;
  const int k = j % W4, yy = j / W4;
  const int xb = 4 * k;
  unsigned am = 0u;
  for (int bc = blockIdx.y; live && bc < BC; bc += gridDim.y) {
    const float* src = dout + (size_t)bc * Ho * Wo;
    float k1 = 1.f, k2 = 0.f, k3 = 0.f;
    if (BN) {
      const int c = bc % C;
      k1 = bn_coef[3 * c]; k2 = bn_coef[3 * c + 1]; k3 = bn_coef[3 * c + 2];
    }
    float g[4] = {0.f, 0.f, 0.f, 0.f};
#pragma unroll
    for (int dy = -1; dy <= 2; ++dy) {
      const int yo = 2 * yy + dy;
      if (yo < 0 || yo >= Ho) continue;
      const float wy = up_w(yo, H, yy);
      if (wy == 0.f) continue;
      const float* row = src + (size_t)yo * Wo + 2 * xb;
      const float4 q0 = *reinterpret_cast<const float4*>(row), q1 = *reinterpret_cast<const float4*>(row + 4);
      float w[10];
      w[0] = xb > 0 ? row[-1] : 0.f;
      w[1] = q0.x; w[2] = q0.y; w[3] = q0.z; w[4] = q0.w; w[5] = q1.x; w[6] = q1.y; w[7] = q1.z; w[8] = q1.w;
      w[9] = 2 * xb + 8 < Wo ? row[8] : 0.f;
      if (BN) {
        const float* yrow = bn_y + (size_t)bc * Ho * Wo + (size_t)yo * Wo + 2 * xb;
        const float4 y0 = *reinterpret_cast<const float4*>(yrow), y1 = *reinterpret_cast<const float4*>(yrow + 4);
        const float v[10] = {xb > 0 ? yrow[-1] : 0.f, y0.x, y0.y, y0.z, y0.w, y1.x, y1.y, y1.z, y1.w, 2 * xb + 8 < Wo ? yrow[8] : 0.f};
#pragma unroll
// ... 677 lines not shown
```

### wt-pse-code_amd/wtpse_hip/nn.py

```python
import math
import os

import torch
import torch.nn as nn

from . import ops


class ConvP(nn.Module):

    def __init__(self, cin, cout, k):
        super().__init__()
        self.cin, self.cout, self.k = cin, cout, k
        self.weight = nn.Parameter(torch.empty(cout, cin, k, k))
        self.bias = nn.Parameter(torch.empty(cout))
        nn.init.kaiming_uniform_(self.weight, a=math.sqrt(5))
        bound = 1.0 / math.sqrt(cin * k * k)
        nn.init.uniform_(self.bias, -bound, bound)
        self.wf_off = self.wd_off = -1
        self.xf_off = self.xd_off = -1
        self.x16f_off = self.x16d_off = -1


class BNP(nn.Module):
# ... 609 lines not shown
        t1, pro1 = Act.parts(a1)
        y, ss, mean, invstd = ops.conv_fwd_bnf(a0.t, t1, wptr, layout, conv.bias, conv.cout, conv.k, a0.pro, _relu_bits(a0, a1), pro1,
                                               bn.weight, bn.bias, bn.running_mean, bn.running_var, bn.num_batches_tracked,
                                               momentum=root.bn_momentum, in_amax0=act_amax(a0) if layout else None,
                                               in_amax1=act_amax(a1) if layout == 1 else None, act_amax=tab)
    else:
        stats_wanted = training or blend is not None
        y, stats = _conv(conv, a0, a1, False, stats_wanted, want_amax=not stats_wanted)
        ss, mean, invstd, tab = _bn_coeffs(root, bn, y, stats, training, tab, getattr(y, "wt_amax", None), want_tape, blend)
    z = Act(y, ss, relu, tab)
    if not want_tape:
        return z, None
    t = Tape()
    t.a0, t.a1, t.y, t.ss, t.mean, t.invstd, t.relu = a0, a1, y, ss, mean, invstd, relu
    t.bn, t.conv, t.frozen = bn, conv, not training
    return z, t


BN_IN = os.environ.get("WTPSE_BN_IN", "1") != "0"
def _bn_bwd(bn, t, dz, root):
    if t.frozen:
        if root.bn_synced:
            raise RuntimeError("frozen BatchNorm statistics are not supported together with synchronised BatchNorm")
        if isinstance(dz, PreBN):
            if dz.coef is not None:
                return ops.bn_bwd_scale_coef(dz.g, dz.coef)
            return ops.bn_bwd_from_stats_frozen(dz.g, dz.stats, bn.weight, t.invstd, root.gview(bn.weight), root.gview(bn.bias),
                                                root.gbias(t.conv))
        return ops.bn_bwd_frozen(dz, t.y, t.ss, t.relu, bn.weight, t.mean, t.invstd, root.gview(bn.weight), root.gview(bn.bias),
                                 root.gbias(t.conv))
    if isinstance(dz, PreBN):
        if dz.coef is not None:
            return ops.bn_bwd_apply_coef(dz.g, t.y, dz.coef)
        return ops.bn_bwd_from_stats(dz.g, t.y, dz.stats, bn.weight, t.mean, t.invstd, root.gview(bn.weight), root.gview(bn.bias))
    if root.bn_synced:
        return root._dp.bn_bwd_synced(dz, t, bn, root)
    return ops.bn_bwd(dz, t.y, t.ss, t.relu, bn.weight, t.mean, t.invstd, root.gview(bn.weight), root.gview(bn.bias))


def convbn_bwd(conv, bn, t, dz, need_dx=True, below0=None, below1=None):
    root = conv._root
    dy = _bn_bwd(bn, t, dz, root)
    _wgrad_side(conv, dy, t.a0, t.a1)
    if not need_dx:
        return None, None
    split = t.a0.t.shape[1] if t.a1 is not None else None
    return _dgrad(conv, dy, split, below0=below0, below1=below1)


def convd_fwd(blk, x, training, want_tape=True):
    t = Tape()
    x = as_act(x)
    t.x = x
    h = x if blk.first else Act(ops.maxpool2_fwd(x.t, x.pro, x.relu), amax=x.amax)
    a, t.c1 = convbn_fwd(blk.conv1, blk.bn1, h, None, False, training, want_tape)
    b, t.c2 = convbn_fwd(blk.conv2, blk.bn2, a, None, True, training, want_tape)
    c, t.c3 = convbn_fwd(blk.conv3, blk.bn3, b, None, True, training, want_tape)
    return c, t


def convd_bwd(blk, t, dz, dx_accum=None, need_dx=True, mask_x=False, below=None):
    d, _ = convbn_bwd(blk.conv3, blk.bn3, t.c3, dz, below0=t.c2)
    d, _ = convbn_bwd(blk.conv2, blk.bn2, t.c2, d, below0=t.c1)
    d, _ = convbn_bwd(blk.conv1, blk.bn1, t.c1, d, need_dx=need_dx)
    if not need_dx:
        return None
    if blk.first:
        if dx_accum is not None:
            ops.axpy(dx_accum, d)
            d = dx_accum
        return ops.relu_mask(d, t.x.t) if mask_x else d
    root = blk.conv1._root
    if (BN_FUSED_STATS and below is not None and below.mean is not None and t.x.relu and t.x.pro is not None
            and not root.bn_synced):
        r = ops.maxpool2_bwd_bnb(t.x.t, d, dx_accum, t.x.pro, t.x.relu, below.mean)
        if r is not None:
            return PreBN(r[0], r[1])
    return ops.maxpool2_bwd(t.x.t, d, dx_accum, dx_accum is not None, t.x.pro, t.x.relu, mask=mask_x)


CONVU_CONV_FIRST = os.environ.get("WTPSE_CONVU_REFERENCE_ORDER", "0") != "1"


def upbn_fwd(conv, bn, a0, training, want_tape=True):
    root = conv._root
    blend = _blend_state(root, training, want_tape)
    stats_wanted = training or blend is not None
    z, _ = _conv(conv, a0, None, False, False, want_amax=not stats_wanted)
    y, stats = ops.upsample2x_fwd_stats(z) if stats_wanted else (ops.upsample2x_fwd(z), None)
    ss, mean, invstd, tab = _bn_coeffs(root, bn, y, stats, training, None, getattr(z, "wt_amax", None), want_tape, blend)
    out = Act(y, ss, True, tab)
    if not want_tape:
        return out, None
    t = Tape()
    t.a0, t.a1, t.y, t.ss, t.mean, t.invstd, t.relu = a0, None, y, ss, mean, invstd, True
    t.bn, t.conv, t.frozen = bn, conv, not training
    return out, t


def upbn_bwd(conv, bn, t, dz, below=None):
    root = conv._root
    if BN_IN and isinstance(dz, PreBN) and dz.coef is not None and dz.g.shape[3] % 8 == 0:
        dzl = ops.upsample2x_bwd_bn(dz.g, t.y, dz.coef)
    else:
        dzl = ops.upsample2x_bwd(_bn_bwd(bn, t, dz, root))
    _wgrad_side(conv, dzl, t.a0, None)
    return _dgrad(conv, dzl, below0=below)[0]


def convu_fwd(blk, x, prev, training, want_tape=True):
    t = Tape()
    x = as_act(x)
    if not blk.first:
        x, t.c1 = convbn_fwd(blk.conv1, blk.bn1, x, None, True, training, want_tape)
    B, _, H, W = x.t.shape
    t.swapped = CONVU_CONV_FIRST and W % 2 == 0 and B * blk.conv2.cout < 32768
    if t.swapped:
        y, t.c2 = upbn_fwd(blk.conv2, blk.bn2, x, training, want_tape)
    else:
        u = Act(ops.upsample2x_fwd(x.t, x.pro, x.relu), amax=x.amax)
        y, t.c2 = convbn_fwd(blk.conv2, blk.bn2, u, None, True, training, want_tape)
    out, t.c3 = convbn_fwd(blk.conv3, blk.bn3, prev, y, True, training, want_tape)
    return out, t


def convu_bwd(blk, t, dout, below_x=None):
    dprev, dy = convbn_bwd(blk.conv3, blk.bn3, t.c3, dout, below1=t.c2)
    if t.swapped:
        dx = upbn_bwd(blk.conv2, blk.bn2, t.c2, dy, below=(below_x if blk.first else t.c1))
    else:
        du, _ = convbn_bwd(blk.conv2, blk.bn2, t.c2, dy)
        dx = ops.upsample2x_bwd(du)
    if not blk.first:
        dx, _ = convbn_bwd(blk.conv1, blk.bn1, t.c1, dx, below0=below_x)
    return dx, dprev


def unet_fwd(net, x1, training, want_tape=True):
    t = Tape()
    x1 = as_act(x1)
    x2, t.d1 = convd_fwd(net.down1, x1, training, want_tape)
    x3, t.d2 = convd_fwd(net.down2, x2, training, want_tape)
    x4, t.d3 = convd_fwd(net.down3, x3, training, want_tape)
    x5, t.d4 = convd_fwd(net.down4, x4, training, want_tape)
    x, t.u1 = convu_fwd(net.up1, x5, x4, training, want_tape)
    x, t.u2 = convu_fwd(net.up2, x, x3, training, want_tape)
    x, t.u3 = convu_fwd(net.up3, x, x2, training, want_tape)
    x, t.u4 = convu_fwd(net.up4, x, x1, training, want_tape)
    return x, t


def unet_bwd(net, t, dfeat, need_dx1=True, decoder_done=None, mask_x=None, below_x1=None):
    d, g1 = convu_bwd(net.up4, t.u4, dfeat, below_x=t.u3.c3)
    d, g2 = convu_bwd(net.up3, t.u3, d, below_x=t.u2.c3)
    d, g3 = convu_bwd(net.up2, t.u2, d, below_x=t.u1.c3)
    g5, g4 = convu_bwd(net.up1, t.u1, d, below_x=t.d4.c3)
    if decoder_done is not None:
        decoder_done()
    g4 = convd_bwd(net.down4, t.d4, g5, g4, below=t.d3.c3)
    g3 = convd_bwd(net.down3, t.d3, g4, g3, below=t.d2.c3)
    g2 = convd_bwd(net.down2, t.d2, g3, g2, below=t.d1.c3)
    g1 = convd_bwd(net.down1, t.d1, g2, g1, mask_x=mask_x is not None, below=below_x1)
    return g1 if need_dx1 else None


def _head_fusable(seq, idxs, x):
    ls = [seq[i] for i in idxs]
    if len(ls) not in (2, 3) or (ls[0].cin, ls[0].cout, ls[1].cin, ls[1].cout) != (32, 32, 32, 8):
        return None
    if len(ls) == 3 and not (ls[2].cin == 8 and 1 <= ls[2].cout <= 4):
        return None
    if any(l.k != 1 for l in ls) or (x.t.shape[2] * x.t.shape[3]) % 32 != 0:
        return None
# ... 119 lines not shown
```

### wt-pse-code_amd/wtpse_hip/ops.py

```python
import torch

from .lib import lib

_WS = {}


_RAW_STREAM = getattr(torch._C, "_cuda_getCurrentRawStream", None)


def stream_ptr():
    if _RAW_STREAM is not None:
        return _RAW_STREAM(torch.cuda.current_device())
    return torch.cuda.current_stream().cuda_stream


def ptr(t):
    return 0 if t is None else t.data_ptr()


def _chk(t, name="tensor"):
    if t is None:
        return
    if not (t.is_cuda and t.dtype == torch.float32 and t.is_contiguous()):
        raise ValueError("%s must be a contiguous fp32 tensor in device memory (got %s, %s, contiguous=%s)"
# ... 265 lines not shown
        tickets, tview = _tickets(L.query("wtpse_bnb_tail_tickets", nblk, cout), dy.device)
        frozen = len(tail) == 5
        args = [ptr(dy), C, wpacked_ptr, layout, ptr(out0), ptr(out1), csplit, ptr(bn_y), ptr(bn_ss), ptr(bn_mean), int(bool(bn_relu)),
                c0, c1, ptr(stats), ptr(gamma), ptr(invstd), ptr(coef), ptr(dgamma), ptr(dbeta)] + ([ptr(tail[4])] if frozen else [])
        _ticket_call(tview, "wtpse_dgrad_bnb_coef_frozen" if frozen else "wtpse_dgrad_bnb_coef", *args, 0, ptr(partial2), tickets,
                     B, H, W, cout, ksize, ptr(in_amax), stream_ptr())
        return out0, out1, stats, coef
    if layout == 2:
        L.call("wtpse_conv16_x3", ptr(dy), C, wpacked_ptr, 0, 0, 0, ptr(out0), ptr(stats), 0, ptr(bn_y), ptr(bn_ss), ptr(bn_mean),
               int(bool(bn_relu)), B, H, W, cout, 0, 1, ptr(in_amax), 0, stream_ptr())
    elif layout == 1:
        L.call("wtpse_dgrad_x3_bnb", ptr(dy), C, wpacked_ptr, ptr(out0), ptr(out1), csplit, ptr(bn_y), ptr(bn_ss), ptr(bn_mean),
               int(bool(bn_relu)), c0, c1, ptr(stats), B, H, W, cout, ksize, ptr(in_amax), stream_ptr())
    else:
        L.call("wtpse_dgrad_bnb", ptr(dy), C, wpacked_ptr, ptr(out0), ptr(out1), csplit,
               ptr(bn_y), ptr(bn_ss), ptr(bn_mean), int(bool(bn_relu)), c0, c1, ptr(stats), B, H, W, cout, ksize, stream_ptr())
    return out0, out1, stats, None


def _wgrad_prelude(query, dy, x0, x1, taps, want_dbias=False):
    _chk(dy, "dy"); _chk(x0, "x0"); _chk(x1, "x1")
    B, cout, H, W = dy.shape
    L, C0, C1 = lib(), x0.shape[1], 0 if x1 is None else x1.shape[1]
    n = L.query(query, B, H, W, C0 + C1, cout)
    slab = workspace("wgrad_slab", n * cout * (C0 + C1) * taps, dy.device)
    dbs = workspace("wgrad_dbias", n * cout, dy.device) if want_dbias else None
    return L, n, slab, dbs, B, cout, H, W, C0, C1


def conv_wgrad(dy, x0, x1, ksize, dw, dbias, pro0=None, pro_relu=0, accumulate=False, pro1=None):
    L, ks, slab, dbs, B, cout, H, W, C0, C1 = _wgrad_prelude("wtpse_wgrad_ksplit", dy, x0, x1, ksize * ksize, dbias is not None)
    L.call("wtpse_conv_wgrad", ptr(dy), ptr(x0), C0, ptr(x1), C1, ptr(pro0), ptr(pro1), int(pro_relu), ptr(slab), ptr(dbs), ks,
           ptr(dw), ptr(dbias), int(accumulate), B, H, W, cout, ksize, stream_ptr())


def wgrad_x3_supported(cin, cout, ksize, c0):
    return bool(lib().query("wtpse_wgrad_x3_supported", int(cin), int(cout), int(ksize), int(c0)))


def conv_wgrad_x3(dy, x0, x1, ksize, dw, pro0=None, pro_relu=0, accumulate=False, pro1=None):
    L, ks, slab, _, B, cout, H, W, C0, C1 = _wgrad_prelude("wtpse_wgrad_x3_ksplit", dy, x0, x1, ksize * ksize)
    L.call("wtpse_conv_wgrad_x3", ptr(dy), ptr(x0), C0, ptr(x1), C1, ptr(pro0), ptr(pro1), int(pro_relu), ptr(slab), ks, ptr(dw),
           int(accumulate), B, H, W, cout, ksize, stream_ptr())


def wgrad_r_supported(cin, cout, ksize, c0, w):
    return bool(lib().query("wtpse_wgrad_r_supported", int(cin), int(cout), int(ksize), int(c0), int(w)))


def conv_wgrad_r(dy, x0, x1, dw, dbias=None, pro0=None, pro_relu=0, accumulate=False, pro1=None, dy_amax=None, x_amax0=None,
                 x_amax1=None):
    L, ns, slab, dbs, B, cout, H, W, C0, C1 = _wgrad_prelude("wtpse_wgrad_r_slabs", dy, x0, x1, 9, dbias is not None)
    L.call("wtpse_conv_wgrad_r", ptr(dy), ptr(x0), C0, ptr(x1), C1, ptr(pro0), ptr(pro1), int(pro_relu), ptr(slab), ptr(dbs), ns,
           ptr(dw), ptr(dbias), int(accumulate), B, H, W, cout, ptr(dy_amax), ptr(x_amax0), ptr(x_amax1), stream_ptr())


def conv_wgrad_r_bn(g, bn_y, coef, x0, x1, dw, pro0=None, pro_relu=0, accumulate=False, pro1=None):
    _chk(bn_y, "bn_y")
    L, ns, slab, _, B, cout, H, W, C0, C1 = _wgrad_prelude("wtpse_wgrad_r_slabs", g, x0, x1, 9)
    L.call("wtpse_conv_wgrad_r_bn", ptr(g), ptr(bn_y), ptr(coef), ptr(x0), C0, ptr(x1), C1, ptr(pro0), ptr(pro1), int(pro_relu),
           ptr(slab), ns, ptr(dw), int(accumulate), B, H, W, cout, stream_ptr())


def conv_fwd_bnf(in0, in1, wpacked_ptr, layout, bias, cout, ksize, pro0, pro_relu, pro1, gamma, beta, rmean, rvar, nbt,
                 momentum=0.1, eps=1e-5, in_amax0=None, in_amax1=None, act_amax=None):
    _chk(in0, "in0"); _chk(in1, "in1"); _chk(pro0, "pro0"); _chk(pro1, "pro1")
    layout = int(layout)
    B, C0, H, W = in0.shape
    C1 = 0 if in1 is None else in1.shape[1]
    L = lib()
    dev = in0.device
    out = torch.empty((B, cout, H, W), dtype=torch.float32, device=dev)
    nblk = _stats_blocks(layout, B, H, W, cout, ksize)
    stats = torch.empty((nblk, cout, 2), dtype=torch.float32, device=dev)
    ss = torch.empty((cout, 2), dtype=torch.float32, device=dev)
    mean = torch.empty((cout,), dtype=torch.float32, device=dev)
    invstd = torch.empty((cout,), dtype=torch.float32, device=dev)
    partial2 = torch.empty(L.query("wtpse_bnb_tail_partial2", nblk, cout), dtype=torch.float64, device=dev)
    tickets, tview = _tickets(L.query("wtpse_bnb_tail_tickets", nblk, cout), dev)
    _ticket_call(tview, "wtpse_conv_fwd_bnf", ptr(in0), C0, ptr(in1), C1, wpacked_ptr, layout, ptr(bias), ptr(pro0), ptr(pro1), int(pro_relu),
           ptr(out), ptr(stats), ptr(gamma), ptr(beta), ptr(rmean), ptr(rvar), ptr(nbt), float(momentum), float(eps), ptr(ss),
           ptr(mean), ptr(invstd), ptr(partial2), tickets, B, H, W, cout, ksize, ptr(in_amax0), ptr(in_amax1), ptr(act_amax),
           stream_ptr())
    return out, ss, mean, invstd


def bn_finalize(stats, count, gamma, beta, rmean, rvar, nbt, momentum=0.1, eps=1e-5, act_amax=None):
    nblk, C, _ = stats.shape
    dev = stats.device
    ss = torch.empty((C, 2), dtype=torch.float32, device=dev)
    mean = torch.empty((C,), dtype=torch.float32, device=dev)
    invstd = torch.empty((C,), dtype=torch.float32, device=dev)
    lib().call("wtpse_bn_finalize", ptr(stats), nblk, C, int(count), ptr(gamma), ptr(beta), ptr(rmean), ptr(rvar),
               ptr(nbt), float(momentum), float(eps), ptr(ss), ptr(mean), ptr(invstd), ptr(act_amax), stream_ptr())
    return ss, mean, invstd


def bn_finalize_blend(stats, count, gamma, beta, rmean, rvar, w, eps=1e-5, acc=None, acc_count=0, moments=None, div=None, act_amax=None):
    nblk, C, _ = stats.shape
    for t, shape in ((acc, (C, 2)), (moments, (C, 4)), (div, (C,))):
        if t is not None and not (t.is_cuda and t.dtype == torch.float64 and t.is_contiguous() and tuple(t.shape) == shape):
            raise ValueError("bn_finalize_blend: acc / moments / div must be contiguous float64 device tensors [C,2] / [C,4] / [C]")
    ss = torch.empty((C, 2), dtype=torch.float32, device=stats.device)
    lib().call("wtpse_bn_finalize_blend", ptr(stats), nblk, C, int(count), ptr(gamma), ptr(beta), ptr(rmean), ptr(rvar), float(w),
               float(eps), ptr(acc), float(acc_count), ptr(ss), ptr(moments), ptr(div), ptr(act_amax), stream_ptr())
    return ss


def bn_eval_coeffs(gamma, beta, rmean, rvar, eps=1e-5):
    C = gamma.numel()
    ss = torch.empty((C, 2), dtype=torch.float32, device=gamma.device)
    lib().call("wtpse_bn_eval_coeffs", ptr(gamma), ptr(beta), ptr(rmean), ptr(rvar), float(eps), C, ptr(ss), stream_ptr())
    return ss


def bn_eval_coeffs_stats(gamma, beta, rmean, rvar, eps=1e-5):
    C = gamma.numel()
    ss = torch.empty((C, 2), dtype=torch.float32, device=gamma.device)
    mean = torch.empty((C,), dtype=torch.float32, device=gamma.device)
    invstd = torch.empty((C,), dtype=torch.float32, device=gamma.device)
    lib().call("wtpse_bn_eval_coeffs_stats", ptr(gamma), ptr(beta), ptr(rmean), ptr(rvar), float(eps), C, ptr(ss), ptr(mean),
               ptr(invstd), stream_ptr())
    return ss, mean, invstd


def affine_act(y, ss, relu):
    _chk(y, "y")
    B, C, H, W = y.shape
    z = torch.empty_like(y)
    lib().call("wtpse_affine_act", ptr(y), ptr(ss), int(relu), ptr(z), B, C, H * W, stream_ptr())
    return z


def _dy_like(t):
    dy = torch.empty_like(t)
    dy.wt_amax = _amax_table(t.device)
    return dy


def bn_bwd(dz, y, ss, relu, gamma, mean, invstd, dgamma, dbeta, accumulate=False):
    _chk(dz, "dz"); _chk(y, "y")
    B, C, H, W = y.shape
    L = lib()
    ns = L.query("wtpse_bn_bwd_nsplit", B, C, H * W)
    partial = workspace("bn_bwd_partial", ns * C * 2, y.device)
    coef = workspace("bn_bwd_coef", C * 3, y.device)
    dy = _dy_like(y)
    L.call("wtpse_bn_bwd", ptr(dz), ptr(y), ptr(ss), int(relu), ptr(gamma), ptr(mean), ptr(invstd), ptr(partial),
           ptr(coef), ptr(dgamma), ptr(dbeta), int(accumulate), ptr(dy), B, C, H * W, ptr(dy.wt_amax), stream_ptr())
    return dy


def bn_bwd_from_stats(g, y, stats, gamma, mean, invstd, dgamma, dbeta, accumulate=False):
    _chk(g, "g"); _chk(y, "y"); _chk(stats, "stats")
    B, C, H, W = y.shape
    assert stats.shape[1] == C
    coef = workspace("bn_bwd_coef", C * 3, y.device)
    dy = _dy_like(y)
    lib().call("wtpse_bn_bwd_from_stats", ptr(g), ptr(y), ptr(stats), stats.shape[0], ptr(gamma), ptr(mean), ptr(invstd), ptr(coef),
               ptr(dgamma), ptr(dbeta), int(accumulate), ptr(dy), B, C, H * W, ptr(dy.wt_amax), stream_ptr())
    return dy


def bn_bwd_frozen(dz, y, ss, relu, gamma, mean, invstd, dgamma, dbeta, dbias, accumulate=False):
    _chk(dz, "dz"); _chk(y, "y")
    B, C, H, W = y.shape
# ... 815 lines not shown
```

Before: 809.2.

## Fuse 1x1 conv, bilinear 2x upsample and BN statistics into one kernel

Adds an epilogue mode to the fp32 and x2h/x3 1x1 convolution kernels. It stages the conv tile in shared memory, performs the bilinear 2x upsample directly from it, writes the upsampled output, and accumulates BN sum/sumsq for the in-launch BN finalize tail. Tiles overlap by one source row/column so each block can produce complete output quads. This removes the round trip of the pre-upsample activation through global memory and the separate upsample+stats kernel. In exchange it adds halo recomputation, a shared-memory scratch area and new tiling logic, and it is enabled by default for training.

```diff
diff --git a/include/wtpse_hip.h b/include/wtpse_hip.h
--- a/include/wtpse_hip.h
+++ b/include/wtpse_hip.h
@@ -45,6 +45,14 @@
                        const float* beta, float* running_mean, float* running_var, long long* num_batches, float momentum, float eps,
                        float* scale_shift, float* save_mean, float* save_invstd, double* partial2, unsigned* tickets, int B, int H,
                        int W, int Cout, int ksize, const unsigned* in_amax0, const unsigned* in_amax1, unsigned* act_amax, void* stream);
+
+int wtpse_upconv_stats_blocks(int B, int H, int W);
+int wtpse_upconv_tile(int H, int W, int tile, int* r);
+int wtpse_upconv_fwd_bnf(const float* in0, int C0, const void* wpacked, int layout, const float* bias, const float* pro0, int pro_relu,
+                         float* out, float* stats, const float* gamma, const float* beta, float* running_mean, float* running_var,
+                         long long* num_batches, float momentum, float eps, float* scale_shift, float* save_mean,
+                         float* save_invstd, double* partial2, unsigned* tickets, int B, int H, int W, int Cout,
+                         const unsigned* in_amax, unsigned* act_amax, void* stream);
 
 int wtpse_bnb_tail_partial2(int nblk, int Cout);
 int wtpse_bnb_tail_tickets(int nblk, int Cout);
diff --git a/wt-pse-code_amd/wtpse_hip/csrc/conv.hip b/wt-pse-code_amd/wtpse_hip/csrc/conv.hip
--- a/wt-pse-code_amd/wtpse_hip/csrc/conv.hip
+++ b/wt-pse-code_amd/wtpse_hip/csrc/conv.hip
@@ -1,4 +1,5 @@
 #include "internal.h"
+#include "upsample_math.h"
 
 #define WTPSE_P16_KC(KS) ((KS) == 3 ? 4 : 8)
 
@@ -70,7 +71,10 @@
   constexpr int WS_SZ = XP ? 0 : NW * 1024;
   constexpr int GRAM_SZ = (P16 && KS == 3) ? 4 * 16 * 65 + 4 * 256 : 0;
   constexpr int RED_SZ = 4 * CB * 2 > GRAM_SZ ? 4 * CB * 2 : GRAM_SZ;
-  constexpr int MAIN_SZ = (XS_SZ + WS_SZ) > RED_SZ ? (XS_SZ + WS_SZ) : RED_SZ;
+  static_assert(EPI != 3 || (KS == 1 && MODE == 0 && !DB), "the fused upsampling epilogue: 1x1, 16 channels x 256 pixels");
+  constexpr int ZS_SZ = EPI == 3 ? CB * UP_ZP : 0;
+  constexpr int OPS_SZ = (XS_SZ + WS_SZ) > RED_SZ ? (XS_SZ + WS_SZ) : RED_SZ;
+  constexpr int MAIN_SZ = OPS_SZ > ZS_SZ ? OPS_SZ : ZS_SZ;
   __shared__ __attribute__((aligned(16))) float smem[MAIN_SZ + CB + (BNB ? 4 * CB : 0)];
   float* bias_s = smem + MAIN_SZ;
   const float* bnp_s = bias_s + CB;
@@ -93,6 +97,12 @@
   const int HW = a.H * a.W;
   if (tid < CB) bias_s[tid] = (a.bias && cout0 + tid < a.Cout) ? a.bias[cout0 + tid] : 0.f;
   if (BNB && tid < CB) bnb_stage<CB>(bias_s + CB + tid, cout0 + tid, a);
+  int oy = ty * TH, ox = tx * TW;
+  if constexpr (EPI == 3) {
+    const UpTile ut = upconv_tile(a.H, a.W, TW, TH, ty, tx);
+    oy = ut.gy0;
+    ox = ut.gx0;
+  }
 
   int off[NT];
 #pragma unroll
@@ -231,7 +241,7 @@
   for (int i = 0; i < NPOS; ++i) {
     int p = tid + 256 * i;
     int r = p / PITCH, x = p - r * PITCH;
-    int gy = ty * TH + r - PAD, gx = tx * TW + x - PAD;
+    int gy = oy + r - PAD, gx = ox + x - PAD;
     gpos[i] = (p < PE && gy >= 0 && gy < a.H && gx >= 0 && gx < a.W) ? gy * a.W + gx : -1;
   }
 
@@ -336,6 +346,15 @@
 #pragma unroll
         for (int nt = 0; nt < NT; ++nt) acc[mt][nt][r] += bz[mt][r];
   }
+  if constexpr (EPI == 3) {
+    __syncthreads();
+#pragma unroll
+    for (int nt = 0; nt < NT; ++nt)
+#pragma unroll
+      for (int r = 0; r < NACC; ++r) smem[((lane >> 4) * 4 + r) * UP_ZP + wave * 64 + nt * NB + (lane & (NB - 1))] = acc[0][nt][r];
+    up2_tile_epilogue<TWL, CB>(a.out0, a.stats, a.ftail, a.H, a.W, a.Cout, b, ty, tx, cout0, tid, smem, tile, cblk);
+    return;
+  }
 
   const bool want_stats = a.stats != nullptr;
   if (want_stats) __syncthreads();
@@ -553,7 +572,8 @@
 static int launch_fwd(const ConvArgs& a, hipStream_t st) {
   constexpr int CB = (MODE == 0 || MODE == 3 || MODE == 4) ? 16 : 32 * MODE;
   ConvArgs args = a;
-  const Tiling t = conv_tiling(a.B, a.H, a.W);
+  const Tiling t = EPI == 3 ? upconv_tiling(a.B, a.H, a.W) : conv_tiling(a.B, a.H, a.W);
+  const int up = EPI == 3 ? 4 : 1;
   args.tiles_x = t.tiles_x;
   args.tiles_y = t.tiles_y;
   dim3 grid((unsigned)t.tiles, (unsigned)ceil_div(a.CoutP, CB));
@@ -562,13 +582,13 @@
   const bool in_launch = tail_in_launch((long long)grid.x * grid.y);
   if (!in_launch) args.tail.tickets = args.ftail.tickets = nullptr;
   if (args.tail.tickets) bnb_tail_geometry(args.tail, (int)grid.x, a.Cout, (double)a.B * a.H * a.W);
-  if (args.ftail.tickets) bnf_tail_geometry(args.ftail, (int)grid.x, a.Cout, (double)a.B * a.H * a.W);
+  if (args.ftail.tickets) bnf_tail_geometry(args.ftail, (int)grid.x, a.Cout, (double)a.B * a.H * a.W * up);
   if (t.TW == 16)
     hipLaunchKernelGGL((conv_fwd_k<KS, MODE, 4, DB, EPI>), grid, dim3(256), 0, st, args);
   else
     hipLaunchKernelGGL((conv_fwd_k<KS, MODE, 5, DB, EPI>), grid, dim3(256), 0, st, args);
   const int rc = wtpse_status();
-  return rc == 0 && !in_launch ? tail_after_launch(a, (int)grid.x, st) : rc;
+  return rc == 0 && !in_launch ? tail_after_launch(a, (int)grid.x, st, up) : rc;
 }
 
 extern "C" int wtpse_conv_stats_blocks(int B, int H, int W) { return conv_tiling(B, H, W).tiles; }
@@ -595,9 +615,11 @@
   WTPSE_REQUIRE(!t.tickets || (bnb && t.partial2 && t.gamma && t.invstd && t.coef && t.dgamma && t.dbeta));
   WTPSE_REQUIRE(!f.tickets || (!bnb && c.stats && !c.gram && f.partial2 && f.gamma && f.beta && f.scale_shift && f.save_mean &&
                                f.save_invstd && (f.rmean == nullptr) == (f.rvar == nullptr)));
+  WTPSE_REQUIRE(!c.up2 || ((layout == CONV_X3 || (layout == CONV_FP32 && c.Cout <= 16)) && c.ksize == 1 && !c.in1 && !c.out1 && !c.mask_ref && !bnb && !c.relu_out && !c.out_amax &&
+                           f.tickets && c.W % 2 == 0 && (((uintptr_t)c.out0) & 15) == 0));
   if (layout == CONV_X3) {
     const X3Tiling g = x3_tiling(c.B, c.H, c.W, c.Cout, c.ksize);
-    WTPSE_REQUIRE(!c.gram && !(c.in_amax1 && !c.in1) && ((c.C0 + c.C1 + 15) & ~15) <= (g.mt == 2 && !g.half ? 512 : 256));
+    WTPSE_REQUIRE(!c.gram && !(c.in_amax1 && !c.in1) && ((c.C0 + c.C1 + 15) & ~15) <= (g.mt == 2 && !g.half && !c.up2 ? 512 : 256));
   }
   if (layout == CONV_C16)
     WTPSE_REQUIRE(c.ksize == 3 && c.C0 <= 16 && c.Cout <= 16 && (((uintptr_t)c.w) & 15) == 0 && !c.in1 && !c.pro1);
@@ -616,6 +638,7 @@
   a.B = c.B; a.H = c.H; a.W = c.W; a.C0 = c.C0; a.C1 = c.C1; a.Cin = c.C0 + c.C1; a.CinP = c16 ? 16 : (a.Cin + 3) & ~3;
   a.Cout = c.Cout; a.CoutP = (c.Cout + 15) & ~15; a.Csplit = c.Csplit; a.pro_relu = c.pro_relu; a.relu_out = c.relu_out;
   a.tiles_x = a.tiles_y = 0;
+  if (c.up2) return launch_fwd<1, 0, false, 3>(a, st);
 #define FWD(KS, M, DB) (bnb ? launch_fwd<KS, M, DB, 2>(a, st) : c.mask_ref ? launch_fwd<KS, M, DB, 1>(a, st) : launch_fwd<KS, M, DB, 0>(a, st))
   if (c16) return (g_x3_terms == 2 && (!c.in_is_grad || c.in_amax0)) ? FWD(3, 4, false) : FWD(3, 3, false);
   int mode = c.Cout <= 16 ? 0 : (c.Cout % 64 == 0 ? 2 : 1);
@@ -685,6 +708,23 @@
   t.nbt = num_batches; t.momentum = momentum; t.eps = eps; t.scale_shift = scale_shift; t.save_mean = save_mean;
   t.save_invstd = save_invstd; t.act_amax = act_amax;
   c.B = B; c.H = H; c.W = W; c.Cout = Cout; c.ksize = ksize;
+  return conv_run(c, layout, (hipStream_t)stream);
+}
+
+extern "C" int wtpse_upconv_fwd_bnf(const float* in0, int C0, const void* wpacked, int layout, const float* bias, const float* pro0,
+                                    int pro_relu, float* out, float* stats, const float* gamma, const float* beta,
+                                    float* running_mean, float* running_var, long long* num_batches, float momentum, float eps,
+                                    float* scale_shift, float* save_mean, float* save_invstd, double* partial2, unsigned* tickets,
+                                    int B, int H, int W, int Cout, const unsigned* in_amax, unsigned* act_amax, void* stream) {
+  WTPSE_REQUIRE(stats && gamma && beta && scale_shift && save_mean && save_invstd && partial2 && tickets);
+  ConvCall c;
+  c.in0 = in0; c.C0 = C0; c.w = wpacked; c.bias = bias; c.pro0 = pro0; c.pro_relu = pro_relu;
+  c.out0 = out; c.Csplit = Cout; c.stats = stats; c.in_amax0 = in_amax; c.up2 = 1;
+  BnfTail& t = c.ftail;
+  t.partial2 = partial2; t.tickets = tickets; t.gamma = gamma; t.beta = beta; t.rmean = running_mean; t.rvar = running_var;
+  t.nbt = num_batches; t.momentum = momentum; t.eps = eps; t.scale_shift = scale_shift; t.save_mean = save_mean;
+  t.save_invstd = save_invstd; t.act_amax = act_amax;
+  c.B = B; c.H = H; c.W = W; c.Cout = Cout; c.ksize = 1;
   return conv_run(c, layout, (hipStream_t)stream);
 }
 
diff --git a/wt-pse-code_amd/wtpse_hip/csrc/conv_x3.hip b/wt-pse-code_amd/wtpse_hip/csrc/conv_x3.hip
--- a/wt-pse-code_amd/wtpse_hip/csrc/conv_x3.hip
+++ b/wt-pse-code_amd/wtpse_hip/csrc/conv_x3.hip
@@ -150,6 +150,24 @@
   return g;
 }
 
+Tiling upconv_tiling(int B, int H, int W) {
+  Tiling t = conv_tiling(B, H, W);
+  t.tiles_x = upconv_tiles_x(W, t.TW); t.tiles_y = upconv_tiles_y(H, t.TH); t.tiles = B * t.tiles_x * t.tiles_y;
+  return t;
+}
+extern "C" int wtpse_upconv_stats_blocks(int B, int H, int W) {
+  WTPSE_REQUIRE(B > 0 && H > 0 && W >= 2 && W % 2 == 0);
+  return upconv_tiling(B, H, W).tiles;
+}
+extern "C" int wtpse_upconv_tile(int H, int W, int tile, int* r) {
+  WTPSE_REQUIRE(r && H > 0 && W >= 2 && W % 2 == 0 && tile >= 0);
+  const Tiling g = upconv_tiling(1, H, W);
+  WTPSE_REQUIRE(tile < g.tiles);
+  const UpTile t = upconv_tile(H, W, g.TW, g.TH, tile / g.tiles_x, tile % g.tiles_x);
+  r[0] = g.tiles_x; r[1] = g.tiles_y; r[2] = t.gy0; r[3] = t.gx0; r[4] = t.p_lo; r[5] = t.p_hi; r[6] = t.k_lo; r[7] = t.k_hi;
+  return 0;
+}
+
 extern "C" int wtpse_conv_x3_stats_blocks(int B, int H, int W, int Cout, int ksize) { return x3_tiling(B, H, W, Cout, ksize).t.tiles; }
 
 int conv_launch_x3(const ConvCall& c, hipStream_t st) {
@@ -167,6 +185,10 @@
   X3Launch L;
   L.g = x3_tiling(c.B, c.H, c.W, c.Cout, c.ksize);
   L.ksize = c.ksize; L.epi = bnb ? 2 : c.mask_ref ? 1 : 0; L.x3r = g_x3r; L.xcd = g_x3_xcd;
+  if (c.up2) {
+    L.g.mt = 1; L.g.px = 256; L.g.half = L.g.small = 0; L.g.t = upconv_tiling(c.B, c.H, c.W);
+    L.epi = 3;
+  }
   return g_x3_terms == 1 ? x3_dispatch_t1(a, L, st) : g_x3_terms == 2 ? x3_dispatch_t2(a, L, st) : x3_dispatch_t3(a, L, st);
 }
 
diff --git a/wt-pse-code_amd/wtpse_hip/csrc/conv_x3_kernels.h b/wt-pse-code_amd/wtpse_hip/csrc/conv_x3_kernels.h
--- a/wt-pse-code_amd/wtpse_hip/csrc/conv_x3_kernels.h
+++ b/wt-pse-code_amd/wtpse_hip/csrc/conv_x3_kernels.h
@@ -2,6 +2,7 @@
 
 #include <stdlib.h>
 #include "internal.h"
+#include "upsample_math.h"
 #include <utility>
 
 typedef __bf16 bf16x8 __attribute__((ext_vector_type(8)));
@@ -318,9 +319,31 @@
   }
 }
 
+template <int TWL>
+__device__ __forceinline__ void x3_up_epilogue(const ConvX3Args& a, f32x16 (&acc)[1][2], int b, int ty, int tx, int cout0, int tid,
+                                               float* zs, const float* bias_s, int tile, int cblk) {
+  constexpr int NACC = 16;
+  const int lane = tid & 63, wave = __builtin_amdgcn_readfirstlane(tid >> 6);
+  const int r32 = lane & 31, h = lane >> 5;
+  if (a.bias) {
+#pragma unroll
+    for (int r = 0; r < NACC; ++r) {
+      const float bz = bias_s[(r & 3) + 8 * (r >> 2) + 4 * h];
+#pragma unroll
+      for (int nt = 0; nt < 2; ++nt) acc[0][nt][r] += bz;
+    }
+  }
+#pragma unroll
+  for (int nt = 0; nt < 2; ++nt)
+#pragma unroll
+    for (int r = 0; r < NACC; ++r) zs[((r & 3) + 8 * (r >> 2) + 4 * h) * UP_ZP + wave * 64 + nt * 32 + r32] = acc[0][nt][r];
+  up2_tile_epilogue<TWL, 32>(a.out0, a.stats, a.ftail, a.H, a.W, a.Cout, b, ty, tx, cout0, tid, zs, tile, cblk);
+}
+
 template <int KS, int MT, int TWL, int EPI, int NT = 2, int TERMS = 3>
 __global__ __launch_bounds__(256, 2) void conv_x3_k(ConvX3Args a) {
   static_assert(TERMS >= 1 && TERMS <= 3, "three bf16 terms (x3), two fp16 terms (x2h) or one bf16 term (bf16 mode)");
+  static_assert(EPI != 3 || (KS == 1 && MT == 1 && NT == 2), "the fused upsampling epilogue: 1x1, 32 channels x 256 pixels");
   constexpr int TAPS = KS * KS, PAD = KS / 2;
   constexpr int TW = 1 << TWL, TH = (128 * NT) / TW;
   constexpr int PITCH = TW + 2 * PAD, ROWS = TH + 2 * PAD;
@@ -333,7 +356,9 @@
   constexpr int WS_U4 = KS * 2 * TERMS * CB;
   constexpr int NW = (WS_U4 + 255) / 256;
   constexpr int RED_F = 4 * CB * 2;
-  constexpr int MAIN_U4 = (XS_U4 + 2 * WS_U4) > (RED_F + 3) / 4 ? (XS_U4 + 2 * WS_U4) : (RED_F + 3) / 4;
+  constexpr int OPS_U4 = (XS_U4 + 2 * WS_U4) > (RED_F + 3) / 4 ? (XS_U4 + 2 * WS_U4) : (RED_F + 3) / 4;
+  constexpr int ZS_U4 = EPI == 3 ? CB * UP_ZP / 4 : 0;
+  constexpr int MAIN_U4 = OPS_U4 > ZS_U4 ? OPS_U4 : ZS_U4;
   constexpr int PRO_MAX = MT == 1 ? 256 : 512;
   __shared__ u32x4v smem[MAIN_U4 + CB / 4 + (EPI == 2 ? CB : 0)];
   __shared__ float2 pro_s[PRO_MAX];
@@ -354,6 +379,12 @@
   const int HW = a.H * a.W;
   if (tid < CB) bias_s[tid] = (a.bias && cout0 + tid < a.Cout) ? a.bias[cout0 + tid] : 0.f;
   if (EPI == 2 && tid < CB) bnb_stage<CB>(bias_s + CB + tid, cout0 + tid, a);
+  int oy = ty * TH, ox = tx * TW;
+  if constexpr (EPI == 3) {
+    const UpTile ut = upconv_tile(a.H, a.W, TW, TH, ty, tx);
+    oy = ut.gy0;
+    ox = ut.gx0;
+  }
 
   float sx = 1.f;
 
@@ -375,7 +406,7 @@
     const int p = (blk - ihalf[i] * PB) * 64 + lane;
     ipos[i] = (blk < 2 * PB && p < PE) ? p : -1;
     const int r = p / PITCH, x = p - r * PITCH;
-    const int gy = ty * TH + r - PAD, gx = tx * TW + x - PAD;
+    const int gy = oy + r - PAD, gx = ox + x - PAD;
     iin[i] = ipos[i] >= 0 && gy >= 0 && gy < a.H && gx >= 0 && gx < a.W;
     voff[i] = iin[i] ? (unsigned)(gy * a.W + gx) * 4u + (unsigned)ihalf[i] * 8u * (unsigned)HW * 4u : BUF_OOB;
   }
@@ -592,7 +623,8 @@
     }
   }
   x3_unscale<TERMS, MT, NT>(a, acc, sx);
-  x3_epilogue<MT, NT, TWL, EPI, true>(a, acc, b, ty, tx, cout0, tid, reinterpret_cast<float*>(smem), bias_s, tile, cblk, true);
+  if constexpr (EPI == 3) x3_up_epilogue<TWL>(a, acc, b, ty, tx, cout0, tid, reinterpret_cast<float*>(smem), bias_s, tile, cblk);
+  else x3_epilogue<MT, NT, TWL, EPI, true>(a, acc, b, ty, tx, cout0, tid, reinterpret_cast<float*>(smem), bias_s, tile, cblk, true);
 }
 
 
@@ -833,7 +865,15 @@
   const bool in_launch = tail_in_launch((long long)grid.x * grid.y);
   if (!in_launch) args.tail.tickets = args.ftail.tickets = nullptr;
   if (args.tail.tickets) bnb_tail_geometry(args.tail, (int)grid.x, a.Cout, (double)a.B * a.H * a.W);
-  if (args.ftail.tickets) bnf_tail_geometry(args.ftail, (int)grid.x, a.Cout, (double)a.B * a.H * a.W);
+  if (args.ftail.tickets) bnf_tail_geometry(args.ftail, (int)grid.x, a.Cout, (double)a.B * a.H * a.W * (EPI == 3 ? 4 : 1));
+  if constexpr (EPI == 3) {
+    if constexpr (KS == 1 && MT == 1) {
+      if (narrow) hipLaunchKernelGGL((conv_x3_k<1, 1, 4, 3, 2, TERMS>), grid, dim3(256), 0, st, args);
+      else hipLaunchKernelGGL((conv_x3_k<1, 1, 5, 3, 2, TERMS>), grid, dim3(256), 0, st, args);
+    }
+    const int rc = wtpse_status();
+    return rc == 0 && !in_launch ? tail_after_launch(a, (int)grid.x, st, 4) : rc;
+  } else
   if (KS == 3 && (L.x3r == 2 || (L.x3r == 1 && MT == 2))) {
     if constexpr (KS == 3) {
       const bool plain = !a.pro0 && !a.pro1 && !a.pro_relu;
@@ -877,6 +917,7 @@
 template <int TERMS>
 static int x3_dispatch(const ConvX3Args& a, const X3Launch& L, hipStream_t st) {
 #define X3E(KS, M) (L.epi == 2 ? launch_x3<KS, M, 2, TERMS>(a, L, st) : L.epi == 1 ? launch_x3<KS, M, 1, TERMS>(a, L, st) : launch_x3<KS, M, 0, TERMS>(a, L, st))
+  if (L.epi == 3) return launch_x3<1, 1, 3, TERMS>(a, L, st);
   if (L.ksize == 3) return L.g.mt == 2 ? X3E(3, 2) : X3E(3, 1);
   return L.g.mt == 2 ? X3E(1, 2) : X3E(1, 1);
 #undef X3E
diff --git a/wt-pse-code_amd/wtpse_hip/csrc/internal.h b/wt-pse-code_amd/wtpse_hip/csrc/internal.h
--- a/wt-pse-code_amd/wtpse_hip/csrc/internal.h
+++ b/wt-pse-code_amd/wtpse_hip/csrc/internal.h
@@ -28,6 +28,7 @@
   BnbTail tail = bnb_tail_none();
   BnfTail ftail = bnf_tail_none();
   int B = 0, H = 0, W = 0, Cout = 0, ksize = 0, relu_out = 0;
+  int up2 = 0;
 };
 enum { CONV_FP32 = 0, CONV_X3 = 1, CONV_C16 = 2 };
 WTPSE_INTERNAL int conv_run(const ConvCall& c, int layout, hipStream_t st);
@@ -51,6 +52,7 @@
   Tiling t;
 };
 WTPSE_INTERNAL X3Tiling x3_tiling(int B, int H, int W, int Cout, int ksize);
+WTPSE_INTERNAL Tiling upconv_tiling(int B, int H, int W);
 
 struct WgradCall {
   const float* dy = nullptr;
@@ -83,10 +85,10 @@
   return workgroups <= max_wgs;
 }
 template <class Args>
-static inline int tail_after_launch(const Args& a, int nblk, hipStream_t stream) {
+static inline int tail_after_launch(const Args& a, int nblk, hipStream_t stream, int up = 1) {
   const BnbTail& tl = a.tail;
   const BnfTail& fl = a.ftail;
-  const long long count = (long long)a.B * a.H * a.W;
+  const long long count = (long long)a.B * a.H * a.W * up;
   if (tl.tickets && tl.dbias)
     return wtpse_bn_bwd_finalize_coef_frozen(a.stats, nblk, a.bn_c1 - a.bn_c0, tl.gamma, tl.invstd, tl.coef, tl.dgamma, tl.dbeta,
                                              tl.dbias, tl.accumulate, stream);
diff --git a/wt-pse-code_amd/wtpse_hip/csrc/pointwise.hip b/wt-pse-code_amd/wtpse_hip/csrc/pointwise.hip
--- a/wt-pse-code_amd/wtpse_hip/csrc/pointwise.hip
+++ b/wt-pse-code_amd/wtpse_hip/csrc/pointwise.hip
@@ -1,4 +1,5 @@
 #include "common.h"
+#include "upsample_math.h"
 
 __device__ __forceinline__ float act_in(float v, const float* pro, int c, int relu) {
   if (pro) v = fmaf(v, pro[2 * c], pro[2 * c + 1]);
@@ -137,14 +138,6 @@
   g = (accumulate & 1) ? dx[i] + g : g;
   if ((accumulate & 2) && !(act_in(x[i], pro, c, relu) > 0.f)) g = 0.f;
   dx[i] = g;
-}
-
-__device__ __forceinline__ void up_src(int d, int n, int& i0, int& i1, float& l1) {
-  float s = 0.5f * (d + 0.5f) - 0.5f;
-  if (s < 0.f) s = 0.f;
-  i0 = (int)s;
-  i1 = i0 + (i0 < n - 1 ? 1 : 0);
-  l1 = s - (float)i0;
 }
 
 __global__ __launch_bounds__(256) void upsample2x_fwd_k(const float* __restrict__ x, const float* __restrict__ pro, int relu,
@@ -201,21 +194,8 @@
     const float* r1 = x + (size_t)bc * H * W + (size_t)y1 * W;
     float a[4] = {act_in(r0[xm1], pro, c, relu), act_in(r0[m], pro, c, relu), act_in(r0[x1], pro, c, relu), act_in(r0[x2], pro, c, relu)};
     float b[4] = {act_in(r1[xm1], pro, c, relu), act_in(r1[m], pro, c, relu), act_in(r1[x1], pro, c, relu), act_in(r1[x2], pro, c, relu)};
-    float ha[4], hb[4];
-    if (m == 0) { ha[0] = fmaf(0.f, a[2], a[1]); hb[0] = fmaf(0.f, b[2], b[1]); }
-    else        { ha[0] = fmaf(0.25f, a[0], 0.75f * a[1]); hb[0] = fmaf(0.25f, b[0], 0.75f * b[1]); }
-    ha[1] = fmaf(0.25f, a[2], 0.75f * a[1]); hb[1] = fmaf(0.25f, b[2], 0.75f * b[1]);
-    ha[2] = fmaf(0.25f, a[1], 0.75f * a[2]); hb[2] = fmaf(0.25f, b[1], 0.75f * b[2]);
-    ha[3] = fmaf(0.25f, a[3], 0.75f * a[2]); hb[3] = fmaf(0.25f, b[3], 0.75f * b[2]);
     float4 oa, ob;
-    oa.x = fmaf(1.f - la, ha[0], la * hb[0]);
-    oa.y = fmaf(1.f - la, ha[1], la * hb[1]);
-    oa.z = fmaf(1.f - la, ha[2], la * hb[2]);
-    oa.w = fmaf(1.f - la, ha[3], la * hb[3]);
-    ob.x = fmaf(1.f - lb, ha[0], lb * hb[0]);
-    ob.y = fmaf(1.f - lb, ha[1], lb * hb[1]);
-    ob.z = fmaf(1.f - lb, ha[2], lb * hb[2]);
-    ob.w = fmaf(1.f - lb, ha[3], lb * hb[3]);
+    up2_quad(a, b, m == 0, la, lb, oa, ob);
     float* ob0 = out + (size_t)bc * Ho * Wo + 4 * k;
     if (va) *reinterpret_cast<float4*>(ob0 + (size_t)ya * Wo) = oa;
     if (vb) *reinterpret_cast<float4*>(ob0 + (size_t)yb * Wo) = ob;
diff --git a/wt-pse-code_amd/wtpse_hip/csrc/upsample_math.h b/wt-pse-code_amd/wtpse_hip/csrc/upsample_math.h
--- /dev/null
+++ b/wt-pse-code_amd/wtpse_hip/csrc/upsample_math.h
@@ -0,0 +1,119 @@
+#pragma once
+#include "common.h"
+
+__device__ __forceinline__ void up_src(int d, int n, int& i0, int& i1, float& l1) {
+  float s = 0.5f * (d + 0.5f) - 0.5f;
+  if (s < 0.f) s = 0.f;
+  i0 = (int)s;
+  i1 = i0 + (i0 < n - 1 ? 1 : 0);
+  l1 = s - (float)i0;
+}
+
+__device__ __forceinline__ void up2_quad(const float (&a)[4], const float (&b)[4], bool first, float la, float lb, float4& oa,
+                                         float4& ob) {
+  float ha[4], hb[4];
+  if (first) { ha[0] = fmaf(0.f, a[2], a[1]); hb[0] = fmaf(0.f, b[2], b[1]); }
+  else       { ha[0] = fmaf(0.25f, a[0], 0.75f * a[1]); hb[0] = fmaf(0.25f, b[0], 0.75f * b[1]); }
+  ha[1] = fmaf(0.25f, a[2], 0.75f * a[1]); hb[1] = fmaf(0.25f, b[2], 0.75f * b[1]);
+  ha[2] = fmaf(0.25f, a[1], 0.75f * a[2]); hb[2] = fmaf(0.25f, b[1], 0.75f * b[2]);
+  ha[3] = fmaf(0.25f, a[3], 0.75f * a[2]); hb[3] = fmaf(0.25f, b[3], 0.75f * b[2]);
+  oa.x = fmaf(1.f - la, ha[0], la * hb[0]);
+  oa.y = fmaf(1.f - la, ha[1], la * hb[1]);
+  oa.z = fmaf(1.f - la, ha[2], la * hb[2]);
+  oa.w = fmaf(1.f - la, ha[3], la * hb[3]);
+  ob.x = fmaf(1.f - lb, ha[0], lb * hb[0]);
+  ob.y = fmaf(1.f - lb, ha[1], lb * hb[1]);
+  ob.z = fmaf(1.f - lb, ha[2], lb * hb[2]);
+  ob.w = fmaf(1.f - lb, ha[3], lb * hb[3]);
+}
+
+struct UpTile {
+  int gy0, gx0;
+  int p_lo, p_hi;
+  int k_lo, k_hi;
+};
+__host__ __device__ __forceinline__ int upconv_tiles_y(int H, int TH) { return H <= TH ? 1 : (H + 1 + TH - 2) / (TH - 1); }
+__host__ __device__ __forceinline__ int upconv_tiles_x(int W, int TW) { return W <= TW ? 1 : (W / 2 + TW / 2 - 2) / (TW / 2 - 1); }
+__host__ __device__ __forceinline__ UpTile upconv_tile(int H, int W, int TW, int TH, int ty, int tx) {
+  UpTile t;
+  if (H <= TH) {
+    t.gy0 = 0; t.p_lo = -1; t.p_hi = H - 1;
+  } else {
+    t.p_lo = ty * (TH - 1) - 1;
+    t.p_hi = t.p_lo + TH - 2 < H - 1 ? t.p_lo + TH - 2 : H - 1;
+    t.gy0 = t.p_lo > 0 ? t.p_lo : 0;
+  }
+  if (W <= TW) {
+    t.gx0 = 0; t.k_lo = 0; t.k_hi = W / 2 - 1;
+  } else {
+    t.k_lo = tx * (TW / 2 - 1);
+    t.k_hi = t.k_lo + TW / 2 - 2 < W / 2 - 1 ? t.k_lo + TW / 2 - 2 : W / 2 - 1;
+    t.gx0 = t.k_lo > 0 ? 2 * t.k_lo - 1 : 0;
+  }
+  return t;
+}
+
+constexpr int UP_ZP = 256;
+template <int TWL, int CB>
+__device__ __forceinline__ void up2_tile_epilogue(float* __restrict__ out, float* __restrict__ stats, const BnfTail& ftail, int H, int W,
+                                                  int Cout, int b, int ty, int tx, int cout0, int tid, float* zs, int tile, int cblk) {
+  constexpr int TW = 1 << TWL, TH = 256 >> TWL;
+  constexpr int QL = TW / 2, PL = 64 / QL, NCH = CB / 4;
+  static_assert(CB % 4 == 0 && CB * UP_ZP >= 524, "four waves share the channels; the fold's scratch (256 doubles + flag) aliases zs");
+  const int lane = tid & 63, wave = __builtin_amdgcn_readfirstlane(tid >> 6);
+  __syncthreads();
+  const int Ho = 2 * H, Wo = 2 * W;
+  const UpTile t = upconv_tile(H, W, TW, TH, ty, tx);
+  const int k = t.k_lo + (lane & (QL - 1));
+  const bool kin = k <= t.k_hi;
+  const int m = 2 * k;
+  const int xm1 = kin ? max(m - 1, 0) - t.gx0 : 0, x0 = kin ? m - t.gx0 : 0;
+  const int x1 = kin ? min(m + 1, W - 1) - t.gx0 : 0, x2 = kin ? min(m + 2, W - 1) - t.gx0 : 0;
+  const int c_w = cout0 + wave * NCH;
+  const float* zw = zs + wave * NCH * UP_ZP;
+  float* ow = out + ((size_t)b * Cout + c_w) * (size_t)Ho * Wo + 4 * k;
+  const size_t plane = (size_t)Ho * Wo;
+  float sv[2 * NCH];
+#pragma unroll
+  for (int i = 0; i < 2 * NCH; ++i) sv[i] = 0.f;
+  for (int p = t.p_lo + lane / QL; p <= t.p_hi; p += PL) {
+    const int ya = 2 * p + 1, yb = 2 * p + 2;
+    const bool va = kin && ya >= 0, vb = kin && yb < Ho;
+    int t0, t1;
+    float la = 0.f, lb = 0.f;
+    if (ya >= 0) up_src(ya, H, t0, t1, la);
+    if (yb < Ho) up_src(yb, H, t0, t1, lb);
+    const int y0 = max(p, 0) - t.gy0, y1 = (p < 0 ? min(1, H - 1) : min(p + 1, H - 1)) - t.gy0;
+    const float* r0 = zw + y0 * TW;
+    const float* r1 = zw + y1 * TW;
+    float* oa_p = ow + (size_t)max(ya, 0) * Wo;
+    float* ob_p = ow + (size_t)min(yb, Ho - 1) * Wo;
+#pragma unroll
+    for (int j = 0; j < NCH; ++j) {
+      if (c_w + j < Cout) {
+        const float ra[4] = {r0[j * UP_ZP + xm1], r0[j * UP_ZP + x0], r0[j * UP_ZP + x1], r0[j * UP_ZP + x2]};
+        const float rb[4] = {r1[j * UP_ZP + xm1], r1[j * UP_ZP + x0], r1[j * UP_ZP + x1], r1[j * UP_ZP + x2]};
+        float4 oa, ob;
+        up2_quad(ra, rb, m == 0, la, lb, oa, ob);
+        if (va) *reinterpret_cast<float4*>(oa_p + j * plane) = oa;
+        if (vb) *reinterpret_cast<float4*>(ob_p + j * plane) = ob;
+        sv[2 * j] += (va ? (oa.x + oa.y) + (oa.z + oa.w) : 0.f) + (vb ? (ob.x + ob.y) + (ob.z + ob.w) : 0.f);
+        sv[2 * j + 1] += (va ? (oa.x * oa.x + oa.y * oa.y) + (oa.z * oa.z + oa.w * oa.w) : 0.f) +
+                         (vb ? (ob.x * ob.x + ob.y * ob.y) + (ob.z * ob.z + ob.w * ob.w) : 0.f);
+      }
+    }
+  }
+#pragma unroll
+  for (int msk = 1; msk < 64; msk <<= 1)
+#pragma unroll
+    for (int i = 0; i < 2 * NCH; ++i) sv[i] += __shfl_xor(sv[i], msk, 64);
+  {
+    float mine = 0.f;
+#pragma unroll
+    for (int i = 0; i < 2 * NCH; ++i) mine = lane == i ? sv[i] : mine;
+    const int c = c_w + (lane >> 1);
+    if (lane < 2 * NCH && c < Cout) pub_store(stats + ((size_t)tile * Cout + c) * 2 + (lane & 1), mine);
+  }
+  const TailTicket tk = bnf_tail_begin(ftail, tile, cblk, tid);
+  bnf_tail<CB>(tk, ftail, stats, Cout, cout0, tile, cblk, tid, reinterpret_cast<double*>(zs), reinterpret_cast<int*>(zs + 520));
+}
diff --git a/wt-pse-code_amd/wtpse_hip/nn.py b/wt-pse-code_amd/wtpse_hip/nn.py
--- a/wt-pse-code_amd/wtpse_hip/nn.py
+++ b/wt-pse-code_amd/wtpse_hip/nn.py
@@ -715,13 +715,31 @@
 CONVU_CONV_FIRST = os.environ.get("WTPSE_CONVU_REFERENCE_ORDER", "0") != "1"
 
 
+UPCONV_FUSED = os.environ.get("WTPSE_UPCONV_FUSED", "1") != "0"
+
+
+def upconv_fused(conv, a0, training, root):
+    if not (UPCONV_FUSED and training) or root.bn_synced:
+        return False
+    B, C0, H, W = a0.t.shape
+    return ops.upconv_supported(_weights(conv)[0], C0, conv.cout, H, W)
+
+
 def upbn_fwd(conv, bn, a0, training, want_tape=True):
     root = conv._root
+    a0 = as_act(a0)
     blend = _blend_state(root, training, want_tape)
     stats_wanted = training or blend is not None
-    z, _ = _conv(conv, a0, None, False, False, want_amax=not stats_wanted)
-    y, stats = ops.upsample2x_fwd_stats(z) if stats_wanted else (ops.upsample2x_fwd(z), None)
-    ss, mean, invstd, tab = _bn_coeffs(root, bn, y, stats, training, None, getattr(z, "wt_amax", None), want_tape, blend)
+    if upconv_fused(conv, a0, training, root):
+        tab = ops.fwd_amax_table(a0.t.device)
+        layout, wptr = _weights(conv)
+        y, ss, mean, invstd = ops.upconv_fwd_bnf(a0.t, wptr, layout, conv.bias, conv.cout, a0.pro, _relu_bits(a0, None), bn.weight,
+                                                 bn.bias, bn.running_mean, bn.running_var, bn.num_batches_tracked,
+                                                 momentum=root.bn_momentum, in_amax=act_amax(a0) if layout else None, act_amax=tab)
+    else:
+        z, _ = _conv(conv, a0, None, False, False, want_amax=not stats_wanted)
+        y, stats = ops.upsample2x_fwd_stats(z) if stats_wanted else (ops.upsample2x_fwd(z), None)
+        ss, mean, invstd, tab = _bn_coeffs(root, bn, y, stats, training, None, getattr(z, "wt_amax", None), want_tape, blend)
     out = Act(y, ss, True, tab)
     if not want_tape:
         return out, None
diff --git a/wt-pse-code_amd/wtpse_hip/ops.py b/wt-pse-code_amd/wtpse_hip/ops.py
--- a/wt-pse-code_amd/wtpse_hip/ops.py
+++ b/wt-pse-code_amd/wtpse_hip/ops.py
@@ -371,6 +371,33 @@
            ptr(out), ptr(stats), ptr(gamma), ptr(beta), ptr(rmean), ptr(rvar), ptr(nbt), float(momentum), float(eps), ptr(ss),
            ptr(mean), ptr(invstd), ptr(partial2), tickets, B, H, W, cout, ksize, ptr(in_amax0), ptr(in_amax1), ptr(act_amax),
            stream_ptr())
+    return out, ss, mean, invstd
+
+
+def upconv_supported(layout, C0, cout, H, W):
+    layout = int(layout)
+    return (layout == 1 and C0 <= 256 or layout == 0 and cout <= 16) and W >= 2 and W % 2 == 0 and H >= 1
+
+
+def upconv_fwd_bnf(in0, wpacked_ptr, layout, bias, cout, pro0, pro_relu, gamma, beta, rmean, rvar, nbt, momentum=0.1, eps=1e-5,
+                   in_amax=None, act_amax=None):
+    _chk(in0, "in0"); _chk(pro0, "pro0")
+    B, C0, H, W = in0.shape
+    L = lib()
+    dev = in0.device
+    out = torch.empty((B, cout, 2 * H, 2 * W), dtype=torch.float32, device=dev)
+    nblk = L.query("wtpse_upconv_stats_blocks", B, H, W)
+    if nblk <= 0:
+        raise ValueError("wtpse_upconv_fwd_bnf does not take a %d x %d map" % (H, W))
+    stats = torch.empty((nblk, cout, 2), dtype=torch.float32, device=dev)
+    ss = torch.empty((cout, 2), dtype=torch.float32, device=dev)
+    mean = torch.empty((cout,), dtype=torch.float32, device=dev)
+    invstd = torch.empty((cout,), dtype=torch.float32, device=dev)
+    partial2 = torch.empty(L.query("wtpse_bnb_tail_partial2", nblk, cout), dtype=torch.float64, device=dev)
+    tickets, tview = _tickets(L.query("wtpse_bnb_tail_tickets", nblk, cout), dev)
+    _ticket_call(tview, "wtpse_upconv_fwd_bnf", ptr(in0), C0, wpacked_ptr, int(layout), ptr(bias), ptr(pro0), int(pro_relu), ptr(out), ptr(stats),
+                 ptr(gamma), ptr(beta), ptr(rmean), ptr(rvar), ptr(nbt), float(momentum), float(eps), ptr(ss), ptr(mean), ptr(invstd),
+                 ptr(partial2), tickets, B, H, W, cout, ptr(in_amax), ptr(act_amax), stream_ptr())
     return out, ss, mean, invstd
 
 
```

Result: no change. 808.2 (median of 2 runs) (-0.1%).
